# bdsaglam/torch-scae

Hardware: AMD Instinct MI355X
Metric: images/sec SCAE fwd+bwd, MNIST 40x40 bs=128, 1/2/4/8 MI355X (higher is better)
Workload: dtype f32

## Files before the change

include/scae_hip.h:

```cpp
#ifndef SCAE_HIP_H
#define SCAE_HIP_H

#include <stdint.h>

#ifdef __cplusplus
extern "C" {
#endif

#define SCAE_ABI_VERSION 3

#define SCAE_OK 0
#define SCAE_ERR_BAD_ARG (-1)
#define SCAE_ERR_UNSUPPORTED (-2)

#define SCAE_MAX_CHANNELS 4
#define SCAE_ATTN_MAX_SET 64
#define SCAE_RENDER_MAX_TEMPLATE_ELEMS 4096

int scae_abi_version(void);
const char *scae_error_string(int code);

void *scae_launch_list_begin(void *stream);
int scae_launch_list_end(void *list);
int scae_launch_list_size(const void *list);
// ... 30 lines not shown
                               float *gq, float *gk, float *gv,
                               float *gpresence, int HB, int N, int M, int dk,
                               int dv, float sqrt_dk, void *stream);

int scae_set_encoder_param_count(int D, int Din, int Dout, int L, int layer_norm);
int scae_set_encoder_grid(int B);
int scae_set_encoder_supported(int N, int D, int Din, int Dout, int L, int layer_norm);
int scae_set_encoder_fwd_f32(int nseg, const float *const *seg_ptr, const int *seg_width,
                             const int *seg_row_stride, const int64_t *seg_batch_stride,
                             const float *presence, const float *params, float *z,
                             float *hsave, int B, int N, int D, int Din, int Dout, int L,
                             int layer_norm, void *stream);
int scae_set_encoder_bwd_f32(int nseg, const float *const *seg_ptr, const int *seg_width,
                             const int *seg_row_stride, const int64_t *seg_batch_stride,
                             float *const *seg_grad, const float *presence,
                             const float *params, const float *hsave, const float *gz,
                             float *pg_partial, int B, int N, int D, int Din, int Dout,
                             int L, int layer_norm, void *stream);
int scae_set_encoder_bf16_supported(int N, int D, int Din, int Dout, int L, int layer_norm);
int scae_set_encoder_fwd_bf16(int nseg, const float *const *seg_ptr, const int *seg_width,
                              const int *seg_row_stride, const int64_t *seg_batch_stride,
                              const float *presence, const float *params, float *z,
                              float *hsave, int B, int N, int D, int Din, int Dout, int L,
                              int layer_norm, void *stream);
int scae_set_encoder_bwd_bf16(int nseg, const float *const *seg_ptr, const int *seg_width,
                              const int *seg_row_stride, const int64_t *seg_batch_stride,
                              float *const *seg_grad, const float *presence,
                              const float *params, const float *hsave, const float *gz,
                              float *pg_partial, int B, int N, int D, int Din, int Dout,
                              int L, int layer_norm, void *stream);

int scae_seed_attention_splits(int B, int O);
int scae_seed_attention_grid(int B, int O);
int scae_seed_attention_supported(int N, int O, int D, int C);
int scae_seed_attention_fwd_f32(const float *h, const float *q, const float *wk,
                                const float *bk, const float *wv, const float *bv,
                                const float *presence, float *out, float *probs, int B,
                                int N, int O, int D, int C, void *stream);
int scae_seed_attention_bwd_f32(const float *h, const float *q, const float *wk,
                                const float *bk, const float *wv, const float *bv,
                                const float *presence, const float *gout, float *gh,
                                float *partial, int B, int N, int O, int D, int C,
                                void *stream);

int scae_seed_attention_mfma_supported(int N, int O, int D, int C);
int scae_seed_attention_mfma_rows(int B);
int scae_seed_attention_mfma_fwd_f32(const float *h, const float *q, const float *wk,
                                     const float *wv, const float *bv, const float *presence,
                                     float *out, int B, int N, int O, int C, void *stream);
int scae_seed_attention_mfma_bwd_f32(const float *h, const float *q, const float *wk,
                                     const float *wv, const float *presence, const float *gout,
                                     float *gh, float *partial, int B, int N, int O, int C,
                                     void *stream);
int scae_seed_attention_mfma_fwd_bf16(const float *h, const float *q, const float *wk,
                                      const float *wv, const float *bv, const float *presence,
                                      float *out, int B, int N, int O, int C, void *stream);
int scae_seed_attention_mfma_bwd_bf16(const float *h, const float *q, const float *wk,
                                      const float *wv, const float *presence,
                                      const float *gout, float *gh, float *partial, int B,
                                      int N, int O, int C, void *stream);
int scae_seed_attention_mfma_reduce_f32(const float *partial, int rows, const float *q,
                                        const float *wk, float *gq, float *gwk, float *gbk,
                                        float *gwv, float *gbv, int O, int C, void *stream);

typedef struct scae_seed_fold_desc {
  const float *seeds;
  const float *wq, *bq, *wk, *bk, *wv, *bv, *wo, *bo;
  const float *w2, *b2;
  float *q, *wkf, *bkf, *wvf, *bvf;
  float *wv2e;
  float *wowv;
  int O, C, D;
} scae_seed_fold_desc;
typedef struct scae_seed_fold_grads {
  const float *g_q, *g_wkf, *g_bkf, *g_wvf, *g_bvf;
  float *d_seeds, *d_wq, *d_bq, *d_wk, *d_bk, *d_wv, *d_bv, *d_wo, *d_bo, *d_w2, *d_b2;
  float *gv2e, *t1;
} scae_seed_fold_grads;
int scae_seed_fold_supported(int O, int C, int D);
int scae_seed_fold_fwd_f32(const scae_seed_fold_desc *desc, void *stream);
int scae_seed_fold_bwd_f32(const scae_seed_fold_desc *desc, const scae_seed_fold_grads *grads,
                           void *stream);

int scae_layer_norm_rows(int64_t rows);
int scae_layer_norm_fwd_f32(const float *x, const float *weight, const float *bias, float *y,
                            float *mean, float *rstd, int64_t rows, int d, float eps,
                            void *stream);
int scae_layer_norm_bwd_f32(const float *x, const float *weight, const float *mean,
                            const float *rstd, const float *gy, float *gx, float *partial,
                            int64_t rows, int d, void *stream);

int scae_gemm_f32(const float *A, const float *B, float *C, const float *bias,
                  const float *mask, float *asum, int batch, int M, int N, int K,
                  int a_kcontig, int lda, int64_t a_batch, int b_kcontig, int ldb,
                  int64_t b_batch, int ldc, int64_t c_batch, int bias_ld, int64_t bias_batch,
                  int ldmask, int64_t mask_batch, int64_t asum_batch, int asum_ld, int relu,
                  void *stream);

typedef struct scae_gemm_desc {
  const float *A, *B;
  float *C;
  const float *bias, *mask;
  float *asum;
  int batch, M, N, K;
  int a_kcontig, lda;
  int64_t a_batch;
  int b_kcontig, ldb;
  int64_t b_batch;
  int ldc;
  int64_t c_batch;
  int bias_ld;
  int64_t bias_batch;
  int ldmask;
  int64_t mask_batch, asum_batch;
  int relu, asum_ld;
  float *c_nomask;
} scae_gemm_desc;
int scae_gemm_pair_f32(const scae_gemm_desc *first, const scae_gemm_desc *second, void *stream);
int scae_gemm_multi_f32(const scae_gemm_desc *descs, int n, void *stream);
int scae_seed_attention_mfma_bwd_gemm_f32(const float *h, const float *q, const float *wk,
                                          const float *wv, const float *presence,
                                          const float *gout, float *gh, float *partial, int B,
                                          int N, int O, int C, const scae_gemm_desc *descs,
                                          int n, void *stream);
int scae_seed_attention_mfma_bwd_gemm_bf16(const float *h, const float *q, const float *wk,
                                           const float *wv, const float *presence,
                                           const float *gout, float *gh, float *partial, int B,
                                           int N, int O, int C, const scae_gemm_desc *descs,
                                           int n, void *stream);


typedef struct scae_mlp_chain_layer {
  const float *w;
  int64_t w_gs;
  int ldw, K, N;
  const float *bias;
  int64_t bias_gs;
  int bias_ld;
  const float *gate;
  int64_t gate_gs, gate_bs;
  float *out;
  int64_t out_gs, out_bs;
  int relu;
} scae_mlp_chain_layer;
typedef struct scae_mlp_chain_desc {
  scae_mlp_chain_layer layer[4];
  int n_layers;
  const float *in;
  int64_t in_gs, in_bs;
  int in_dim, B, G;
  int row_tile;
  int bf16;
} scae_mlp_chain_desc;
int scae_mlp_chain_max_width(void);
int scae_mlp_chain_fwd_f32(const scae_mlp_chain_desc *desc, void *stream);
int scae_mlp_chain_bwd_f32(const scae_mlp_chain_desc *desc, void *stream);

typedef struct scae_votes_desc {
  const float *all_param;
  const float *cpr_static, *bias_cvr, *bias_caps, *bias_vote, *bias_scale;
  const float *noise_caps, *noise_vote;
  float noise_scale;
  int V, ld_param, similarity, learn_vote_scale, allow_deformations;
  float *vote, *scale, *vote_presence, *logit_caps, *logit_vote, *reg_partial;
  float *caps_presence;
  int *caps_arg;
  const float *gvote, *gscale, *gvote_presence, *glogit_caps, *glogit_vote, *greg;
  const float *gcaps_presence;
  float *gall_param, *gcpr_in, *gall_param_gated;
} scae_votes_desc;
int scae_mlp_chain_votes_fwd_f32(const scae_mlp_chain_desc *desc, const scae_votes_desc *votes,
                                 void *stream);
int scae_mlp_chain_votes_bwd_f32(const scae_mlp_chain_desc *desc, const scae_votes_desc *votes,
                                 void *stream);

int scae_gemm_bf16(const float *A, const float *B, float *C, const float *bias,
                   const float *mask, float *asum, int batch, int M, int N, int K,
                   int a_kcontig, int lda, int64_t a_batch, int b_kcontig, int ldb,
                   int64_t b_batch, int ldc, int64_t c_batch, int bias_ld, int64_t bias_batch,
                   int ldmask, int64_t mask_batch, int64_t asum_batch, int asum_ld, int relu,
                   void *stream);
int scae_gemm_pair_bf16(const scae_gemm_desc *first, const scae_gemm_desc *second, void *stream);
int scae_gemm_multi_bf16(const scae_gemm_desc *descs, int n, void *stream);
int scae_conv3x3_fwd_fold_f32(const float *in, const float *wf, const float *bias, float *out,
                              const float *post_bias, float *out_post, int B, int IH, int IW,
                              int Cin, int Cout, int stride, const scae_seed_fold_desc *fold,
                              void *stream);
int scae_conv3x3_fwd_res_supported(int B, int IH, int IW, int Cin, int Cout, int stride);
int scae_conv3x3_fwd_res_f32(const float *in, const float *wp, const float *bias, float *out,
                             const float *post_bias, float *out_post, int B, int IH, int IW,
                             int Cin, int Cout, int stride, int group, void *stream);
int scae_conv3x3_fwd_bf16(const float *in, const float *wf, const float *bias, float *out,
                          const float *post_bias, float *out_post, int B, int IH, int IW, int Cin,
                          int Cout, int stride, void *stream);
int scae_conv3x3_bwd_pair_bf16(const float *dpre, const float *wd, const float *in, float *din,
                               float *partial, int B, int IH, int IW, int Cin, int Cout,
                               int stride, void *stream);

int64_t scae_conv3x3_wf_floats(int Cout, int Cin);
int scae_conv3x3_relayout_f32(const float *w, float *wf, float *wd, int Cout, int Cin,
                              void *stream);

int scae_conv3x3_bf16r_supported(int B, int IH, int IW, int Cin, int Cout, int stride);
int scae_conv3x3_first_fwd_relayout_bf16(const float *img, const float *w, const float *bias,
                                         uint16_t *out_h, int B, int Cin, int IH, int IW,
                                         int Cout, int stride, int n_layers,
                                         const float *const *rw, float *const *rwf,
                                         float *const *rwd, uint16_t *const *rwfh,
                                         uint16_t *const *rwdh, const int *rCout,
                                         const int *rCin, void *stream);
int scae_cvt_bf16_batch(int n_arrays, const float *const *src, uint16_t *const *dst,
                        const int64_t *n, void *stream);
int scae_conv3x3_fwd_bf16r(const uint16_t *in, const uint16_t *wf, const float *bias,
                           uint16_t *out_h, float *out_f, const float *post_bias,
                           float *out_post, int B, int IH, int IW, int Cin, int Cout, int stride,
                           void *stream);
int scae_conv3x3_dgrad_bf16r(const uint16_t *dpre, const uint16_t *wd, const uint16_t *gate,
                             uint16_t *din_h, float *din_f, int B, int IH, int IW, int Cin,
                             int Cout, int stride, void *stream);
int scae_conv3x3_wgrad_bf16r_splits(int B, int OH, int OW, int Cin, int Cout);
int scae_conv3x3_wgrad_bf16r(const uint16_t *dpre, const uint16_t *x, float *partial, int B,
                             int IH, int IW, int Cin, int Cout, int stride, void *stream);
int scae_conv3x3_relayout_batch_f32(int n_layers, const float *const *w, float *const *wf,
                                    float *const *wd, const int *Cout, const int *Cin,
                                    void *stream);
int scae_conv3x3_first_fwd_f32(const float *img, const float *w, const float *bias,
                               float *out, int B, int Cin, int IH, int IW, int Cout,
                               int stride, void *stream);
int scae_conv3x3_first_wgrad_rows(int B, int Cout);
int scae_conv3x3_first_wgrad_f32(const float *dpre, const float *img, float *partial, int B,
                                 int Cin, int IH, int IW, int Cout, int stride, void *stream);
int scae_conv3x3_first_fwd_relayout_f32(const float *img, const float *w, const float *bias,
                                        float *out, int B, int Cin, int IH, int IW, int Cout,
                                        int stride, int n_layers, const float *const *rw,
                                        float *const *rwf, float *const *rwd, const int *rCout,
                                        const int *rCin, void *stream);
int scae_conv3x3_first_wgrad_reduce_f32(const float *dpre, const float *img, float *partial,
                                        int B, int Cin, int IH, int IW, int Cout, int stride,
                                        int n_layers, const float *const *rpartial,
                                        float *const *rdw, float *const *rdb, const int *rCout,
                                        const int *rCin, const int *rsplits, void *stream);
int scae_conv3x3_fwd_f32(const float *in, const float *wf, const float *bias, float *out,
                         const float *post_bias, float *out_post, int B, int IH, int IW,
                         int Cin, int Cout, int stride, void *stream);
int scae_conv3x3_dgrad_f32(const float *dpre, const float *wd, const float *gate, float *din,
                           int B, int IH, int IW, int Cin, int Cout, int stride, void *stream);
int scae_conv3x3_bwd_pair_f32(const float *dpre, const float *wd, const float *in, float *din,
                              float *partial, int B, int IH, int IW, int Cin, int Cout,
                              int stride, void *stream);
int scae_conv3x3_bwd_pair_reduce_f32(const float *dpre, const float *wd, const float *in,
                                     float *din, float *partial, int B, int IH, int IW, int Cin,
                                     int Cout, int stride, const float *rpartial, int rows,
                                     const float *q, const float *wk, float *gq, float *gwk,
                                     float *gbk, float *gwv, float *gbv, int O, int C,
                                     void *stream);
int scae_conv3x3_bwd_pair_fold_f32(const float *dpre, const float *wd, const float *in,
                                   float *din, float *partial, int B, int IH, int IW, int Cin,
                                   int Cout, int stride, const scae_seed_fold_desc *fold,
                                   const scae_seed_fold_grads *fold_grads, void *stream);
int scae_conv3x3_wgrad_splits(int B, int OH, int OW, int Cin, int Cout);
int scae_conv3x3_wgrad_f32(const float *dpre, const float *in, float *partial, float *dw,
                           float *db, int B, int IH, int IW, int Cin, int Cout, int stride,
                           void *stream);
int scae_conv3x3_wgrad_reduce_batch_f32(int n_layers, const float *const *partial,
                                        float *const *dw, float *const *db, const int *Cout,
                                        const int *Cin, const int *splits, void *stream);

int scae_attention_pool_supported(int HW, int A, int P);
int scae_attention_pool_fwd_f32(const float *y, float *out, int B, int HW, int A, int P,
                                void *stream);
int scae_attention_pool_bwd_f32(const float *y, const float *g, float *dy, int B, int HW,
                                int A, int P, void *stream);
int scae_capsule_head_fwd_f32(const float *y, const float *noise_u, float noise_scale,
                              int similarity, float *pooled, float *pose, float *presence,
                              float *feature, float *absence, int B, int HW, int A, int P,
                              void *stream);
int scae_capsule_head_conv_supported(int HW, int A, int P, int C);
int scae_capsule_head_conv_preferred(int B, int HW, int A, int P, int C);
int scae_capsule_head_conv_fwd_f32(const float *x, const float *w, const float *bias, int C,
                                   float *y, const float *noise_u, float noise_scale,
                                   int similarity, float *pooled, float *pose, float *presence,
                                   float *feature, float *absence, int B, int HW, int A, int P,
                                   void *stream);
int scae_capsule_head_conv_fwd_tc_f32(
    const float *x, const float *w, const float *bias, int C, float *y, const float *noise_u,
    float noise_scale, int similarity, float *pooled, float *pose, float *presence,
    float *feature, float *absence, int B, int HW, int A, int P, const float *logits,
    const float *w1, const float *b1, const float *w2, const float *b2, float *raw,
    float *templates, float *color, int Ct, int hw, int F, int H1, int template_nonlin,
    int color_nonlin, void *stream);
int scae_capsule_head_bwd_f32(const float *y, const float *pooled, const float *noise_u,
                              float noise_scale, int similarity, const float *g_pose,
                              const float *g_presence, const float *g_feature,
                              const float *g_feature2, float *dy, int B, int HW, int A, int P,
                              void *stream);
int scae_capsule_head_bwd_tc_f32(
    const float *y, const float *pooled, const float *noise_u, float noise_scale, int similarity,
    const float *g_pose, const float *g_presence, const float *g_feature, float *dy, int B,
    int HW, int A, int P, const float *logits, const float *feature, const float *w1,
    const float *b1, const float *w2, const float *b2, const float *color,
    const float *g_templates, const float *g_raw, float *g_logits, float *tc_g_feature,
    float *partial, int C, int hw, int F, int H1, int template_nonlin, int color_nonlin,
    void *stream);

int scae_rmsprop_step_f32(float *param, const float *grad, float *square_avg, float *buf,
                          int64_t n, float lr, const float *lr_dev, float alpha, float eps,
                          float momentum, float weight_decay, float grad_scale, void *stream);

struct scae_sum_job;
int scae_rmsprop_sums_step_f32(float *param, float *grad, float *square_avg, float *buf,
                               int64_t n, float lr, const float *lr_dev, float alpha, float eps,
                               float momentum, float grad_scale, const struct scae_sum_job *jobs,
                               int n_jobs, void *stream);

#define SCAE_FLAT_OPT_STATE_INTS 2112
int scae_flat_opt_step_f32(float *param, const float *grad, float *exp_avg, float *exp_avg_sq,
                           float *slow, int64_t n, const float *lr_dev, int32_t *step_state,
                           int kind, double beta1, double beta2, float eps, float weight_decay,
                           float grad_scale, int look_ahead_k, float look_ahead_alpha,
                           int advance, void *stream);

int scae_flat_opt_sums_step_f32(float *param, float *grad, float *exp_avg, float *exp_avg_sq,
                                float *slow, int64_t n, const float *lr_dev,
                                int32_t *step_state, int kind, double beta1, double beta2,
                                float eps, float grad_scale, int look_ahead_k,
                                float look_ahead_alpha, const struct scae_sum_job *jobs,
                                int n_jobs, void *stream);

#define SCAE_GRAD_SQ_MAX_PARTIALS 4096
int scae_grad_sq_partials_f32(const float *grad, int64_t n, double *partials, int max_partials,
                              int *n_partials, void *stream);

int scae_grad_sq_partials_sums_f32(float *grad, int64_t n, double *partials, int max_partials,
                                   int *n_partials, const struct scae_sum_job *jobs, int n_jobs,
                                   void *stream);

int scae_rmsprop_clip_step_f32(float *param, const float *grad, float *square_avg, float *buf,
                               int64_t n, float lr, const float *lr_dev, float alpha, float eps,
                               float momentum, float weight_decay, float grad_scale,
                               const double *partials, int n_partials, float max_norm,
                               float *norm_out, void *stream);
int scae_flat_opt_clip_step_f32(float *param, const float *grad, float *exp_avg,
                                float *exp_avg_sq, float *slow, int64_t n, const float *lr_dev,
                                int32_t *step_state, int kind, double beta1, double beta2,
                                float eps, float weight_decay, float grad_scale,
                                int look_ahead_k, float look_ahead_alpha, int advance,
                                const double *partials, int n_partials, float max_norm,
                                float *norm_out, void *stream);

int scae_grad_accumulate_f32(float *acc, const float *grad, int64_t n, void *stream);
int scae_grad_accumulate_sums_f32(float *acc, float *grad, int64_t n,
                                  const struct scae_sum_job *jobs, int n_jobs, void *stream);
int scae_grad_sq_acc_partials_f32(const float *grad, const float *acc, int64_t n,
                                  double *partials, int max_partials, int *n_partials,
                                  void *stream);
int scae_grad_sq_acc_partials_sums_f32(float *grad, const float *acc, int64_t n,
                                       double *partials, int max_partials, int *n_partials,
                                       const struct scae_sum_job *jobs, int n_jobs,
                                       void *stream);
int scae_rmsprop_acc_step_f32(float *param, const float *grad, float *acc, float *square_avg,
                              float *buf, int64_t n, float lr, const float *lr_dev, float alpha,
                              float eps, float momentum, float weight_decay, float grad_scale,
                              void *stream);
int scae_rmsprop_acc_sums_step_f32(float *param, float *grad, float *acc, float *square_avg,
                                   float *buf, int64_t n, float lr, const float *lr_dev,
                                   float alpha, float eps, float momentum, float grad_scale,
                                   const struct scae_sum_job *jobs, int n_jobs, void *stream);
int scae_rmsprop_acc_clip_step_f32(float *param, const float *grad, float *acc,
                                   float *square_avg, float *buf, int64_t n, float lr,
                                   const float *lr_dev, float alpha, float eps, float momentum,
                                   float weight_decay, float grad_scale, const double *partials,
                                   int n_partials, float max_norm, float *norm_out,
                                   void *stream);
int scae_flat_opt_acc_step_f32(float *param, const float *grad, float *acc, float *exp_avg,
                               float *exp_avg_sq, float *slow, int64_t n, const float *lr_dev,
                               int32_t *step_state, int kind, double beta1, double beta2,
                               float eps, float weight_decay, float grad_scale,
                               int look_ahead_k, float look_ahead_alpha, int advance,
                               void *stream);
int scae_flat_opt_acc_sums_step_f32(float *param, float *grad, float *acc, float *exp_avg,
                                    float *exp_avg_sq, float *slow, int64_t n,
                                    const float *lr_dev, int32_t *step_state, int kind,
                                    double beta1, double beta2, float eps, float grad_scale,
                                    int look_ahead_k, float look_ahead_alpha,
                                    const struct scae_sum_job *jobs, int n_jobs, void *stream);
int scae_flat_opt_acc_clip_step_f32(float *param, const float *grad, float *acc,
                                    float *exp_avg, float *exp_avg_sq, float *slow, int64_t n,
                                    const float *lr_dev, int32_t *step_state, int kind,
                                    double beta1, double beta2, float eps, float weight_decay,
                                    float grad_scale, int look_ahead_k, float look_ahead_alpha,
                                    int advance, const double *partials, int n_partials,
                                    float max_norm, float *norm_out, void *stream);

#define SCAE_NORM_CHUNK 2048
#define SCAE_NORM_GROUP_CHUNKS 16
#define SCAE_NORM_INF 0
int scae_segment_norms_chunk(void);
int scae_segment_norms_f32(const float *src, const float *acc, int64_t n, const int32_t *chunks,
                           int n_chunks, const int32_t *group_first, int n_groups,
                           const int32_t *seg_first, int n_segs, int norm_kind, float scale,
                           double *partials, float *ring, int64_t *cursor, int capacity,
                           void *stream);

int scae_stage_batch(float *dst_image, const float *src_image, int64_t n_image,
                     int64_t *dst_label, const int64_t *src_label, int64_t n_label,
                     void *stream);

int scae_step_prologue_f32(float *dst_image, const float *src_image, int64_t n_image,
                           int64_t *dst_label, const int64_t *src_label, int64_t n_label,
                           float *noise, int64_t n_noise, uint64_t *noise_state,
                           const scae_seed_fold_desc *fold, void *stream);

typedef struct scae_first_layer_desc {
  const float *img;
  const float *w;
  const float *bias;
  float *out;
  int B, Cin, IH, IW, Cout, stride;
  int n_layers;
  const float *rw[8];
  float *rwf[8];
  float *rwd[8];
  int rCout[8], rCin[8];
  uint16_t *out_h;
  uint16_t *rwfh[8];
  uint16_t *rwdh[8];
} scae_first_layer_desc;
int scae_step_prologue_first_f32(float *dst_image, const float *src_image, int64_t n_image,
                                 int64_t *dst_label, const int64_t *src_label,
                                 int64_t n_label, float *noise, int64_t n_noise,
                                 uint64_t *noise_state, const scae_seed_fold_desc *fold,
                                 const scae_first_layer_desc *first, void *stream);

typedef struct scae_batch_source_desc {
  const void *images;
  const void *labels;
  const int32_t *index;
  int64_t rows;
  int64_t n;
  int image_u8, label_u8;
  int C, h, w, H, W;
  int shuffle, translate;
  uint64_t seed;
  int64_t epoch, position;
  int rank, world;
  int wrap;
  const int32_t *affine;
  int64_t affine_rows;
} scae_batch_source_desc;
int scae_gather_batch_f32(float *dst_image, int64_t *dst_label, int B,
                          const scae_batch_source_desc *src, void *stream);
int scae_step_prologue_source_f32(float *dst_image, int64_t *dst_label, int B,
                                  const scae_batch_source_desc *src, float *noise,
                                  int64_t n_noise, uint64_t *noise_state,
                                  const scae_seed_fold_desc *fold,
                                  const scae_first_layer_desc *first, void *stream);

int scae_template_color_supported(int M, int C, int F, int H1);
int scae_template_color_partial_rows(int B, int M);
int scae_template_color_fwd_f32(const float *logits, const float *feature, const float *w1,
                                const float *b1, const float *w2, const float *b2, float *raw,
                                float *templates, float *color, int B, int M, int C, int hw,
                                int F, int H1, int template_nonlin, int color_nonlin,
                                void *stream);
int scae_template_color_bwd_f32(const float *logits, const float *feature, const float *w1,
                                const float *b1, const float *w2, const float *b2,
                                const float *color, const float *g_templates,
                                const float *g_raw, float *g_logits, float *g_feature,
                                float *partial, int B, int M, int C, int hw, int F, int H1,
                                int template_nonlin, int color_nonlin, void *stream);

typedef struct scae_sum_segment {
  float *dst;
  int64_t begin, end, period;
} scae_sum_segment;
int scae_sum_rows_f32(const float *src, int64_t rows, int64_t cols,
                      const scae_sum_segment *segments, int n_segments, void *stream);
typedef struct scae_sum_job {
  const float *src;
  int64_t rows, cols;
  const scae_sum_segment *segments;
  int n_segments;
} scae_sum_job;
int scae_sum_rows_multi_f32(const scae_sum_job *jobs, int n_jobs, void *stream);

typedef struct scae_scaled_sum {
  const float *src;
  int64_t n;
  float scale;
  float *dst;
} scae_scaled_sum;
int scae_scaled_sums_f32(const scae_scaled_sum *jobs, int n_jobs, void *stream);

int scae_capsule_votes_fwd_f32(const float *all_param, const float *cpr_static,
                               const float *bias_cvr, const float *bias_caps,
                               const float *bias_vote, const float *bias_scale,
                               const float *noise_caps, const float *noise_vote,
                               float noise_scale, float *vote, float *scale,
                               float *vote_presence, float *logit_caps,
                               float *logit_vote, float *reg_partial,
                               float *caps_presence, int *caps_arg, int B, int O, int V,
                               int ld_param, int similarity, int learn_vote_scale,
                               int allow_deformations, void *stream);
int scae_capsule_votes_bwd_f32(const float *all_param, const float *cpr_static,
                               const float *bias_cvr, const float *bias_caps,
                               const float *bias_vote, const float *bias_scale,
                               const float *noise_caps, const float *noise_vote,
                               float noise_scale, const float *gvote,
                               const float *gscale, const float *gvote_presence,
                               const float *glogit_caps, const float *glogit_vote,
                               const float *greg, const float *gcaps_presence,
                               const int *caps_arg, float *gall_param, float *gcpr_in,
                               float *gall_param_gated, int B, int O, int V, int ld_param,
                               int similarity, int learn_vote_scale,
                               int allow_deformations, void *stream);

int scae_capsule_likelihood_fwd_f32(
    const float *vote, const float *scale, const float *vote_presence,
    const float *dummy_vote, const float *x, const float *presence,
    float *log_prob_per_point, float *vote_presence_binary, float *winner,
    float *winner_presence, int64_t *winner_idx, int64_t *is_from_capsule,
    float *soft_winner, float *soft_winner_presence, float *posterior,
    float *mixing_log_prob, float *mixing_logit, int B, int O, int M,
    void *stream);
int scae_capsule_likelihood_bwd_f32(
    const float *vote, const float *scale, const float *vote_presence,
    const float *dummy_vote, const float *x, const float *presence,
    const float *posterior, const int64_t *winner_idx, const float *g_lpp,
    const float *g_winner, const float *g_winner_presence,
    const float *g_soft_winner, const float *g_soft_winner_presence,
    const float *g_posterior, const float *g_mixing_log_prob,
    const float *g_mixing_logit, float *gvote, float *gscale,
    float *gvote_presence, float *gx, float *gpresence, float *gdummy_partial,
    int B, int O, int M, void *stream);

int scae_class_probs_supported(int O, int ncls);
int scae_class_probs_f32(const float *caps_presence, const float *posterior, const float *w,
                         const float *bias, float *prior_prob, float *post_prob, int B, int O,
                         int M, int ncls, const scae_scaled_sum *extra_sums, int n_extra,
                         void *stream);

typedef struct scae_eval_sink {
  float *rows;
  int64_t capacity;
  int64_t cursor;
  int64_t overflow;
} scae_eval_sink;
#define SCAE_EVAL_RECORD_FLOATS 9
#define SCAE_EVAL_RECORDS_MAX_CLASSES 64
typedef struct scae_eval_records {
  float *rows;
  int64_t capacity;
  int64_t cursor;
  int64_t overflow;
  int64_t *confusion;
  int64_t ncls;
  int64_t labelled;
} scae_eval_records;
#define SCAE_TRAIN_LOG_ROW 19
typedef struct scae_train_log_desc {
  float *rows;
  int64_t *step;
  int capacity;
  double *acc;
  const float *prior_prob, *post_prob;
  const int64_t *label;
  int ncls;
  const float *lr;
} scae_train_log_desc;
typedef struct scae_loss_extras {
  const float *rec_sums;
  int n_rec;
  const float *reg;
  float w_reg;
  float *g_rec_sums, *g_reg;
  float *loss;
  const float *g_loss;
  int defer_combine;
  float *out12;
  const scae_train_log_desc *train_log;
} scae_loss_extras;
int scae_loss_tail_supported(int B, int O, int ncls);
int64_t scae_loss_tail_workspace_floats(int B, int O, int ncls);
int scae_loss_tail_fwd_f32(const float *lpp, const float *posterior,
                           const float *caps_presence, const float *cls_w,
                           const float *cls_b, const int64_t *label,
                           const scae_loss_extras *extras, float *out12, float *workspace,
                           int B, int O, int M, int ncls, int n_classes_cfg, int prior_type,
                           int post_type, int sparsity_on, const float *weights5,
                           float within_const, void *stream);
int scae_loss_tail_defer_preferred(int B, int O);
int scae_loss_tail_combine_f32(const float *lpp, const float *posterior,
                               const float *caps_presence, const float *cls_w,
                               const float *cls_b, const int64_t *label,
                               const scae_loss_extras *extras, float *out12, float *workspace,
                               int B, int O, int M, int ncls, int n_classes_cfg, int prior_type,
                               int post_type, int sparsity_on, const float *weights5,
                               float within_const, void *stream);
int scae_loss_tail_fwd_class_probs_f32(
    const float *lpp, const float *posterior, const float *caps_presence, const float *cls_w,
    const float *cls_b, const int64_t *label, const scae_loss_extras *extras, float *out12,
    float *workspace, int B, int O, int M, int ncls, int n_classes_cfg, int prior_type,
    int post_type, int sparsity_on, const float *weights5, float within_const,
    const float *cp_caps_presence, const float *cp_posterior, const float *cp_w,
    const float *cp_bias, float *prior_prob, float *post_prob, int cp_B, int cp_O, int cp_M,
    int cp_ncls, const scae_scaled_sum *extra_sums, int n_extra, void *stream);
// ... 313 lines not shown
```

torch_scae_amd/_lib.py:

```python
import ctypes
import os
from ctypes import (POINTER, Structure, c_char_p, c_double, c_float, c_int,
                    c_int64, c_uint32, c_uint64, c_void_p)

_HERE = os.path.dirname(os.path.abspath(__file__))
LIB_PATH = os.environ.get("SCAE_HIP_LIB") or os.path.join(_HERE, "lib",
                                                        "libscae_hip.so")

P = c_void_p


class DecoderDesc(Structure):
    _fields_ = [("templates", P), ("templates_alpha", P), ("pose", P),
                ("presence", P), ("bg_image", P), ("bg_value", P),
                ("bg_mixing_logit", P), ("temperature_logit", P),
                ("out_scale", P),
                ("B", c_int), ("M", c_int), ("C", c_int), ("th", c_int),
                ("tw", c_int), ("H", c_int), ("W", c_int),
                ("template_repeat", c_int)]


class LikelihoodBwdDesc(Structure):
    _fields_ = [(n, P) for n in (
        "vote", "scale", "vote_presence", "dummy_vote", "x", "presence",
        "posterior", "winner_idx", "g_lpp", "g_winner", "g_winner_presence",
        "g_soft_winner", "g_soft_winner_presence", "g_posterior",
        "g_mixing_log_prob", "g_mixing_logit", "gvote", "gscale",
        "gvote_presence", "gx", "gpresence", "gdummy_partial")] + [
        ("B", c_int), ("O", c_int), ("M", c_int)]


class GemmDesc(Structure):
    _fields_ = [("A", P), ("B", P), ("C", P), ("bias", P), ("mask", P),
                ("asum", P), ("batch", c_int), ("M", c_int), ("N", c_int),
                ("K", c_int), ("a_kcontig", c_int), ("lda", c_int),
                ("a_batch", c_int64), ("b_kcontig", c_int), ("ldb", c_int),
                ("b_batch", c_int64), ("ldc", c_int), ("c_batch", c_int64),
                ("bias_ld", c_int), ("bias_batch", c_int64), ("ldmask", c_int),
                ("mask_batch", c_int64), ("asum_batch", c_int64),
                ("relu", c_int), ("asum_ld", c_int), ("c_nomask", P)]


class MlpChainLayer(Structure):
    _fields_ = [("w", P), ("w_gs", c_int64), ("ldw", c_int), ("K", c_int),
                ("N", c_int), ("bias", P), ("bias_gs", c_int64),
                ("bias_ld", c_int), ("gate", P), ("gate_gs", c_int64),
                ("gate_bs", c_int64), ("out", P), ("out_gs", c_int64),
                ("out_bs", c_int64), ("relu", c_int)]


class MlpChainDesc(Structure):
    _fields_ = [("layer", MlpChainLayer * 4), ("n_layers", c_int), ("in_", P),
                ("in_gs", c_int64), ("in_bs", c_int64), ("in_dim", c_int),
                ("B", c_int), ("G", c_int), ("row_tile", c_int),
                ("bf16", c_int)]


class VotesDesc(Structure):
    _fields_ = [(n, P) for n in ("all_param", "cpr_static", "bias_cvr",
                                 "bias_caps", "bias_vote", "bias_scale",
                                 "noise_caps", "noise_vote")] + \
        [("noise_scale", c_float), ("V", c_int), ("ld_param", c_int),
         ("similarity", c_int), ("learn_vote_scale", c_int),
         ("allow_deformations", c_int)] + \
        [(n, P) for n in ("vote", "scale", "vote_presence", "logit_caps",
                          "logit_vote", "reg_partial", "caps_presence",
                          "caps_arg", "gvote", "gscale", "gvote_presence",
                          "glogit_caps", "glogit_vote", "greg", "gcaps_presence",
                          "gall_param", "gcpr_in", "gall_param_gated")]


class SumSegment(Structure):
    _fields_ = [("dst", P), ("begin", c_int64), ("end", c_int64),
                ("period", c_int64)]


class SumJob(Structure):
    _fields_ = [("src", P), ("rows", c_int64), ("cols", c_int64),
                ("segments", POINTER(SumSegment)), ("n_segments", c_int)]


class ScaledSum(Structure):
    _fields_ = [("src", P), ("n", c_int64), ("scale", c_float), ("dst", P)]


class TrainLogDesc(Structure):
    _fields_ = [("rows", P), ("step", P), ("capacity", c_int), ("acc", P),
                ("prior_prob", P), ("post_prob", P), ("label", P), ("ncls", c_int),
                ("lr", P)]


class LossExtras(Structure):
    _fields_ = [("rec_sums", P), ("n_rec", c_int), ("reg", P),
                ("w_reg", c_float), ("g_rec_sums", P), ("g_reg", P),
                ("loss", P), ("g_loss", P), ("defer_combine", c_int),
                ("out12", P), ("train_log", POINTER(TrainLogDesc))]


class KMeansDesc(Structure):
    _fields_ = [("x", P), ("N", c_int64), ("F", c_int), ("k", c_int), ("R", c_int),
                ("G", c_int), ("max_iter", c_int), ("centroids", P), ("labels", P),
                ("part_sum", P), ("part_count", P), ("part_changed", P),
                ("part_inertia", P), ("state", P), ("inertia", P)]


class ProbeDesc(Structure):
    _fields_ = [("x", P), ("y", P), ("N", c_int64), ("F", c_int), ("C", c_int), ("R", c_int),
                ("G", c_int), ("max_iter", c_int), ("mean", P), ("scale", P), ("l2", P),
                ("step", P), ("tol", P), ("W", P), ("V", P), ("grad", P), ("t", P),
                ("part_grad", P), ("part_loss", P), ("history", P), ("state", P)]


class TsneDesc(Structure):
    _fields_ = [("N", c_int), ("G", c_int), ("n_iter", c_int), ("exaggeration_iter", c_int),
                ("check_every", c_int), ("early_exaggeration", c_float),
                ("learning_rate", c_float), ("P", P), ("Y", P), ("velocity", P), ("gains", P),
                ("part", P), ("rows", P), ("block", P), ("plogp", P), ("history", P)]


class TsneSparseDesc(Structure):
    _fields_ = [("N", c_int), ("G", c_int), ("n_iter", c_int), ("exaggeration_iter", c_int),
                ("check_every", c_int), ("early_exaggeration", c_float),
                ("learning_rate", c_float), ("indptr", P), ("cols", P), ("vals", P),
                ("nnz", c_int64), ("Y", P), ("velocity", P), ("gains", P), ("part", P),
                ("rows", P), ("block", P), ("plogp", P), ("history", P)]


class SeedFoldDesc(Structure):
    _fields_ = [(n, P) for n in (
        "seeds", "wq", "bq", "wk", "bk", "wv", "bv", "wo", "bo", "w2", "b2",
        "q", "wkf", "bkf", "wvf", "bvf", "wv2e", "wowv")] + \
        [("O", c_int), ("C", c_int), ("D", c_int)]


class FirstLayerDesc(Structure):
    _fields_ = [("img", P), ("w", P), ("bias", P), ("out", P)] + \
        [(n, c_int) for n in ("B", "Cin", "IH", "IW", "Cout", "stride",
                              "n_layers")] + \
        [("rw", P * 8), ("rwf", P * 8), ("rwd", P * 8),
         ("rCout", c_int * 8), ("rCin", c_int * 8),
         ("out_h", P), ("rwfh", P * 8), ("rwdh", P * 8)]


class BatchSourceDesc(Structure):
    _fields_ = [("images", P), ("labels", P), ("index", P), ("rows", c_int64),
                ("n", c_int64)] + \
        [(n, c_int) for n in ("image_u8", "label_u8", "C", "h", "w", "H", "W",
                              "shuffle", "translate")] + \
        [("seed", c_uint64), ("epoch", c_int64), ("position", c_int64),
         ("rank", c_int), ("world", c_int), ("wrap", c_int),
         ("affine", P), ("affine_rows", c_int64)]


class SeedFoldGrads(Structure):
    _fields_ = [(n, P) for n in (
        "g_q", "g_wkf", "g_bkf", "g_wvf", "g_bvf", "d_seeds", "d_wq", "d_bq",
        "d_wk", "d_bk", "d_wv", "d_bv", "d_wo", "d_bo", "d_w2", "d_b2",
        "gv2e", "t1")]


SIGNATURES = {
    "scae_abi_version": [],
    "scae_error_string": [c_int],
    "scae_uniform_f32": [P, c_int64, P, P],
    "scae_geometric_transform_fwd_f32": [P, P, c_int64, c_int, c_int, c_int, P],
    "scae_geometric_transform_bwd_f32": [P, P, P, c_int64, c_int, c_int, c_int,
                                         P],
    "scae_mat3_mul_fwd_f32": [P, P, P, c_int64, c_int, P],
    "scae_mat3_mul_bwd_f32": [P, P, P, P, P, c_int64, c_int, P],
    "scae_qkv_attention_fwd_f32": [P, P, P, P, P, P, c_int, c_int, c_int,
                                   c_int, c_int, c_float, P],
    "scae_qkv_attention_fwd_bf16": [P, P, P, P, P, P, c_int, c_int, c_int,
                                    c_int, c_int, c_float, P],
    "scae_qkv_attention_bwd_f32": [P, P, P, P, P, P, P, P, P, c_int, c_int,
                                   c_int, c_int, c_int, c_float, P],
    "scae_set_encoder_param_count": [c_int] * 5,
    "scae_set_encoder_grid": [c_int],
    "scae_set_encoder_supported": [c_int] * 6,
    "scae_set_encoder_fwd_f32": [c_int, P, P, P, P, P, P, P, P] + [c_int] * 7 + [P],
    "scae_set_encoder_bwd_f32": [c_int, P, P, P, P, P, P, P, P, P, P]
                                + [c_int] * 7 + [P],
    "scae_render_gmm_sums_bwd_likelihood_f32": [P] * 13,
    "scae_set_encoder_fwd_logprob_f32": [c_int, P, P, P, P, P, P, P, P] + [c_int] * 7
                                        + [P] * 6,
    "scae_set_encoder_fwd_logprob_bf16": [c_int, P, P, P, P, P, P, P, P] + [c_int] * 7
                                         + [P] * 6,
    "scae_set_encoder_bf16_supported": [c_int] * 6,
    "scae_set_encoder_fwd_bf16": [c_int, P, P, P, P, P, P, P, P] + [c_int] * 7 + [P],
    "scae_set_encoder_bwd_bf16": [c_int, P, P, P, P, P, P, P, P, P, P]
                                 + [c_int] * 7 + [P],
    "scae_seed_attention_splits": [c_int] * 2,
    "scae_seed_attention_grid": [c_int] * 2,
    "scae_seed_attention_supported": [c_int] * 4,
    "scae_seed_attention_fwd_f32": [P] * 9 + [c_int] * 5 + [P],
    "scae_seed_attention_bwd_f32": [P] * 10 + [c_int] * 5 + [P],
    "scae_seed_attention_mfma_supported": [c_int] * 4,
    "scae_seed_attention_mfma_rows": [c_int],
    "scae_seed_attention_mfma_fwd_f32": [P] * 7 + [c_int] * 4 + [P],
    "scae_seed_attention_mfma_bwd_f32": [P] * 8 + [c_int] * 4 + [P],
    "scae_seed_attention_mfma_fwd_bf16": [P] * 7 + [c_int] * 4 + [P],
    "scae_seed_attention_mfma_bwd_bf16": [P] * 8 + [c_int] * 4 + [P],
    "scae_seed_attention_mfma_bwd_gemm_f32": [P] * 8 + [c_int] * 4
    + [POINTER(GemmDesc), c_int, P],
    "scae_seed_attention_mfma_bwd_gemm_bf16": [P] * 8 + [c_int] * 4
    + [POINTER(GemmDesc), c_int, P],
    "scae_seed_attention_mfma_reduce_f32": [P, c_int] + [P] * 7 + [c_int] * 2 + [P],
    "scae_seed_fold_supported": [c_int] * 3,
    "scae_seed_fold_fwd_f32": [POINTER(SeedFoldDesc), P],
    "scae_seed_fold_bwd_f32": [POINTER(SeedFoldDesc), POINTER(SeedFoldGrads), P],
    "scae_layer_norm_rows": [c_int64],
    "scae_layer_norm_fwd_f32": [P] * 6 + [c_int64, c_int, c_float, P],
    "scae_layer_norm_bwd_f32": [P] * 7 + [c_int64, c_int, P],
    "scae_gemm_f32": [P] * 6 + [c_int] * 6 + [c_int64, c_int, c_int, c_int64,
                                              c_int, c_int64, c_int, c_int64,
                                              c_int, c_int64, c_int64, c_int, c_int,
                                              P],
    "scae_gemm_bf16": [P] * 6 + [c_int] * 6 + [c_int64, c_int, c_int, c_int64,
                                              c_int, c_int64, c_int, c_int64,
                                              c_int, c_int64, c_int64, c_int, c_int,
                                              P],
    "scae_gemm_pair_f32": [POINTER(GemmDesc), POINTER(GemmDesc), P],
    "scae_launch_list_begin": [P],
    "scae_launch_list_end": [P],
    "scae_launch_list_size": [P],
    "scae_launch_list_run": [P, P],
    "scae_launch_list_lane": [P, c_int],
    "scae_launch_list_timeline": [P, P, P, POINTER(c_float), c_int],
    "scae_launch_list_free": [P],
    "scae_gemm_multi_f32": [POINTER(GemmDesc), c_int, P],
    "scae_gemm_multi_bf16": [POINTER(GemmDesc), c_int, P],
    "scae_mlp_chain_max_width": [],
    "scae_mlp_chain_fwd_f32": [POINTER(MlpChainDesc), P],
    "scae_mlp_chain_bwd_f32": [POINTER(MlpChainDesc), P],
    "scae_mlp_chain_votes_fwd_f32": [POINTER(MlpChainDesc), POINTER(VotesDesc), P],
    "scae_mlp_chain_votes_bwd_f32": [POINTER(MlpChainDesc), POINTER(VotesDesc), P],
    "scae_gemm_pair_bf16": [POINTER(GemmDesc), POINTER(GemmDesc), P],
    "scae_conv3x3_wf_floats": [c_int, c_int],
    "scae_conv3x3_relayout_f32": [P, P, P, c_int, c_int, P],
    "scae_conv3x3_bf16r_supported": [c_int] * 6,
    "scae_conv3x3_first_fwd_relayout_bf16": [P] * 4 + [c_int] * 7 + [P] * 8,
    "scae_cvt_bf16_batch": [c_int, P, P, P, P],
    "scae_conv3x3_fwd_bf16r": [P] * 7 + [c_int] * 6 + [P],
    "scae_conv3x3_dgrad_bf16r": [P] * 5 + [c_int] * 6 + [P],
    "scae_conv3x3_wgrad_bf16r_splits": [c_int] * 5,
    "scae_conv3x3_wgrad_bf16r": [P] * 3 + [c_int] * 6 + [P],
    "scae_conv3x3_relayout_batch_f32": [c_int, P, P, P, P, P, P],
    "scae_conv3x3_first_fwd_f32": [P] * 4 + [c_int] * 6 + [P],
    "scae_conv3x3_first_fwd_relayout_f32": [P] * 4 + [c_int] * 7 + [P] * 6,
    "scae_conv3x3_first_wgrad_reduce_f32": [P] * 3 + [c_int] * 7 + [P] * 7,
    "scae_conv3x3_first_wgrad_rows": [c_int] * 2,
    "scae_conv3x3_first_wgrad_f32": [P] * 3 + [c_int] * 6 + [P],
    "scae_conv3x3_fwd_f32": [P] * 6 + [c_int] * 6 + [P],
    "scae_conv3x3_fwd_fold_f32": [P] * 6 + [c_int] * 6 + [POINTER(SeedFoldDesc), P],
    "scae_conv3x3_fwd_res_supported": [c_int] * 6,
    "scae_conv3x3_fwd_res_f32": [P] * 6 + [c_int] * 7 + [P],
    "scae_conv3x3_fwd_bf16": [P] * 6 + [c_int] * 6 + [P],
    "scae_conv3x3_dgrad_f32": [P] * 4 + [c_int] * 6 + [P],
    "scae_conv3x3_bwd_pair_f32": [P] * 5 + [c_int] * 6 + [P],
    "scae_conv3x3_bwd_pair_reduce_f32": [P] * 5 + [c_int] * 6 + [P, c_int] + [P] * 7
    + [c_int] * 2 + [P],
    "scae_conv3x3_bwd_pair_fold_f32": [P] * 5 + [c_int] * 6
    + [POINTER(SeedFoldDesc), POINTER(SeedFoldGrads), P],
    "scae_conv3x3_bwd_pair_bf16": [P] * 5 + [c_int] * 6 + [P],
    "scae_conv3x3_wgrad_reduce_batch_f32": [c_int] + [P] * 7,
    "scae_conv3x3_wgrad_splits": [c_int] * 5,
    "scae_conv3x3_wgrad_f32": [P] * 5 + [c_int] * 6 + [P],
    "scae_attention_pool_supported": [c_int] * 3,
    "scae_attention_pool_fwd_f32": [P, P] + [c_int] * 4 + [P],
    "scae_attention_pool_bwd_f32": [P, P, P] + [c_int] * 4 + [P],
    "scae_stage_batch": [P, P, c_int64, P, P, c_int64, P],
    "scae_step_prologue_f32": [P, P, c_int64, P, P, c_int64, P, c_int64, P,
                               POINTER(SeedFoldDesc), P],
    "scae_step_prologue_first_f32": [P, P, c_int64, P, P, c_int64, P, c_int64,
                                     P, POINTER(SeedFoldDesc),
                                     POINTER(FirstLayerDesc), P],
    "scae_gather_batch_f32": [P, P, c_int, POINTER(BatchSourceDesc), P],
    "scae_step_prologue_source_f32": [P, P, c_int, POINTER(BatchSourceDesc), P, c_int64, P,
                                      POINTER(SeedFoldDesc), POINTER(FirstLayerDesc), P],
    "scae_rmsprop_step_f32": [P, P, P, P, c_int64, c_float, P, c_float, c_float,
                              c_float, c_float, c_float, P],
    "scae_rmsprop_sums_step_f32": [P, P, P, P, c_int64, c_float, P, c_float, c_float,
                                   c_float, c_float, POINTER(SumJob), c_int, P],
    "scae_flat_opt_step_f32": [P, P, P, P, P, c_int64, P, P, c_int, c_double, c_double, c_float,
                               c_float, c_float, c_int, c_float, c_int, P],
    "scae_flat_opt_sums_step_f32": [P, P, P, P, P, c_int64, P, P, c_int, c_double, c_double,
                                    c_float, c_float, c_int, c_float, POINTER(SumJob), c_int, P],
    "scae_grad_sq_partials_f32": [P, c_int64, P, c_int, POINTER(c_int), P],
    "scae_grad_sq_partials_sums_f32": [P, c_int64, P, c_int, POINTER(c_int), POINTER(SumJob),
                                       c_int, P],
    "scae_rmsprop_clip_step_f32": [P, P, P, P, c_int64, c_float, P, c_float, c_float, c_float,
                                   c_float, c_float, P, c_int, c_float, P, P],
    "scae_flat_opt_clip_step_f32": [P, P, P, P, P, c_int64, P, P, c_int, c_double, c_double,
                                    c_float, c_float, c_float, c_int, c_float, c_int, P, c_int,
                                    c_float, P, P],
    "scae_grad_accumulate_f32": [P, P, c_int64, P],
    "scae_grad_accumulate_sums_f32": [P, P, c_int64, POINTER(SumJob), c_int, P],
    "scae_grad_sq_acc_partials_f32": [P, P, c_int64, P, c_int, POINTER(c_int), P],
    "scae_grad_sq_acc_partials_sums_f32": [P, P, c_int64, P, c_int, POINTER(c_int),
                                           POINTER(SumJob), c_int, P],
    "scae_rmsprop_acc_step_f32": [P, P, P, P, P, c_int64, c_float, P, c_float, c_float,
                                  c_float, c_float, c_float, P],
    "scae_rmsprop_acc_sums_step_f32": [P, P, P, P, P, c_int64, c_float, P, c_float, c_float,
                                       c_float, c_float, POINTER(SumJob), c_int, P],
    "scae_rmsprop_acc_clip_step_f32": [P, P, P, P, P, c_int64, c_float, P, c_float, c_float,
                                       c_float, c_float, c_float, P, c_int, c_float, P, P],
    "scae_flat_opt_acc_step_f32": [P, P, P, P, P, P, c_int64, P, P, c_int, c_double, c_double,
                                   c_float, c_float, c_float, c_int, c_float, c_int, P],
    "scae_flat_opt_acc_sums_step_f32": [P, P, P, P, P, P, c_int64, P, P, c_int, c_double,
                                        c_double, c_float, c_float, c_int, c_float,
                                        POINTER(SumJob), c_int, P],
    "scae_flat_opt_acc_clip_step_f32": [P, P, P, P, P, P, c_int64, P, P, c_int, c_double,
                                        c_double, c_float, c_float, c_float, c_int, c_float,
                                        c_int, P, c_int, c_float, P, P],
    "scae_segment_norms_chunk": [],
    "scae_segment_norms_f32": [P, P, c_int64, P, c_int, P, c_int, P, c_int, c_int, c_float,
                               P, P, P, c_int, P],
    "scae_capsule_head_fwd_f32": [P, P, c_float, c_int, P, P, P, P, P] + [c_int] * 4 + [P],
    "scae_capsule_head_conv_supported": [c_int] * 4,
    "scae_capsule_head_conv_preferred": [c_int] * 5,
    "scae_capsule_head_conv_fwd_f32": [P, P, P, c_int, P, P, c_float, c_int, P, P, P, P, P]
    + [c_int] * 4 + [P],
    "scae_capsule_head_conv_fwd_tc_f32": [P, P, P, c_int, P, P, c_float, c_int, P, P, P, P, P]
    + [c_int] * 4 + [P] * 8 + [c_int] * 6 + [P],
    "scae_capsule_head_bwd_f32": [P, P, P, c_float, c_int, P, P, P, P, P] + [c_int] * 4 + [P],
    "scae_capsule_head_bwd_tc_f32": [P, P, P, c_float, c_int, P, P, P, P] + [c_int] * 4
    + [P] * 12 + [c_int] * 6 + [P],
    "scae_template_color_supported": [c_int] * 4,
    "scae_template_color_partial_rows": [c_int] * 2,
    "scae_template_color_fwd_f32": [P] * 9 + [c_int] * 8 + [P],
    "scae_template_color_bwd_f32": [P] * 12 + [c_int] * 8 + [P],
    "scae_sum_rows_f32": [P, c_int64, c_int64, POINTER(SumSegment), c_int, P],
    "scae_sum_rows_multi_f32": [POINTER(SumJob), c_int, P],
    "scae_scaled_sums_f32": [POINTER(ScaledSum), c_int, P],
    "scae_class_probs_supported": [c_int] * 2,
    "scae_class_probs_f32": [P] * 6 + [c_int] * 4 + [POINTER(ScaledSum), c_int, P],
    "scae_capsule_votes_fwd_f32": [P] * 8 + [c_float] + [P] * 8
                                  + [c_int] * 7 + [P],
    "scae_capsule_votes_bwd_f32": [P] * 8 + [c_float] + [P] * 11
                                  + [c_int] * 7 + [P],
    "scae_capsule_likelihood_fwd_f32": [P] * 17 + [c_int] * 3 + [P],
    "scae_capsule_likelihood_bwd_f32": [P] * 22 + [c_int] * 3 + [P],
    "scae_loss_tail_supported": [c_int] * 3,
    "scae_loss_tail_workspace_floats": [c_int] * 3,
    "scae_loss_tail_fwd_f32": [P] * 6 + [POINTER(LossExtras), P, P] + [c_int] * 8
    + [POINTER(c_float), c_float, P],
    "scae_loss_tail_defer_preferred": [c_int] * 2,
    "scae_loss_tail_combine_f32": [P] * 6 + [POINTER(LossExtras), P, P] + [c_int] * 8
    + [POINTER(c_float), c_float, P],
    "scae_loss_tail_fwd_class_probs_f32": [P] * 6 + [POINTER(LossExtras), P, P]
    + [c_int] * 8 + [POINTER(c_float), c_float] + [P] * 6 + [c_int] * 4
    + [POINTER(ScaledSum), c_int, P],
    "scae_loss_tail_bwd_f32": [P] * 6 + [POINTER(LossExtras)] + [P] * 7
    + [c_int] * 8 + [POINTER(c_float), c_float, P],
    "scae_eval_tail_f32": [P] * 6 + [POINTER(LossExtras), P, P] + [c_int] * 8
    + [POINTER(c_float), c_float] + [P] * 5,
    "scae_loss_tail_fwd_class_probs_sink_f32": [P] * 6 + [POINTER(LossExtras), P, P]
    + [c_int] * 8 + [POINTER(c_float), c_float] + [P] * 6 + [c_int] * 4
    + [POINTER(ScaledSum), c_int, P, P],
    "scae_eval_tail_sink_f32": [P] * 6 + [POINTER(LossExtras), P, P] + [c_int] * 8
    + [POINTER(c_float), c_float] + [P] * 6,
    "scae_eval_tail_records_f32": [P] * 6 + [POINTER(LossExtras), P, P] + [c_int] * 8
    + [POINTER(c_float), c_float] + [P] * 7,
    "scae_eval_records_f32": [P] * 6 + [c_int] * 4 + [P, P],
    "scae_eval_accumulate_f32": [P] * 5 + [c_int] * 2 + [P] * 3,
    "scae_train_log_f32": [P] * 3 + [POINTER(TrainLogDesc), c_int, P],
    "scae_eval_features_f32": [P, P, c_int, c_int, c_int, P, P],
    "scae_kmeans_supported": [c_int] * 2,
    "scae_kmeans_groups": [c_int64, c_int],
    "scae_kmeans_lloyd_f32": [POINTER(KMeansDesc), c_int, P],
    "scae_kmeans_pp_f32": [P, c_int64, c_int, c_int, c_int, c_uint32, P, P, P, P],
    "scae_kmeans_assign_f32": [P, c_int64, c_int, c_int, P, P, P],
    "scae_kmeans_contingency": [P, P, c_int64, c_int, c_int, P, P, P],
    "scae_probe_supported": [c_int] * 3,
    "scae_probe_groups": [c_int64, c_int],
    "scae_probe_predict_blocks": [c_int64],
    "scae_probe_moments_f64": [P, P, c_int64, c_int, c_int, P, P, P, P],
    "scae_probe_fit_f32": [POINTER(ProbeDesc), c_int, P],
    "scae_probe_predict_f32": [P, c_int64, c_int, c_int] + [P] * 8,
    "scae_tsne_supported": [c_int] * 2,
    "scae_tsne_groups": [c_int],
    "scae_tsne_affinities_f32": [P, c_int, c_int, c_float, P, P, P, P, P],
    "scae_tsne_run_f32": [POINTER(TsneDesc), c_int, c_int, P],
    "scae_tsne_sparse_supported": [c_int] * 3,
    "scae_tsne_sparse_groups": [c_int],
    "scae_tsne_knn_bandwidths_f32": [P, c_int, c_int, c_float, P, P, P],
    "scae_tsne_sparse_run_f32": [POINTER(TsneSparseDesc), c_int, c_int, P],
    "scae_knn_wide_f32": [P, c_int64, c_int, c_int, P, P, P, P],
    "scae_knn_supported": [c_int64, c_int64, c_int, c_int],
    "scae_knn_groups": [c_int64, c_int64],
    "scae_knn_f32": [P, c_int64, P, c_int64, c_int, c_int, c_int, P, P, P, P],
    "scae_knn_vote_f32": [P, P, c_int64, c_int, P, c_int64, POINTER(c_int), c_int, c_int, P, P],
    "scae_knn_ranks_f32": [P, c_int64, c_int, P, c_int, P, P, P, P, P],
    "scae_cluster_quality_supported": [c_int64, c_int, c_int64],
    "scae_cluster_quality_labels": [P, c_int64, c_int64, P, P, P],
    "scae_cluster_quality_silhouette_f32": [P, P, P, P, c_int64, c_int, c_int64] + [P] * 7,
    "scae_cluster_quality_dispersion_f32": [P, P, c_int64, c_int, c_int64, P, P],
    "scae_template_render_fwd_f32": [POINTER(DecoderDesc), P, P, P],
    "scae_render_gmm_logprob_fwd_f32": [POINTER(DecoderDesc), P, P, P, P, P],
    "scae_render_gmm_bwd_f32": [POINTER(DecoderDesc)] + [P] * 12 + [P],
    "scae_render_gmm_logprob_tiles": [POINTER(DecoderDesc)],
    "scae_render_gmm_forms": [POINTER(DecoderDesc), c_int, P, P, POINTER(c_int)],
    "scae_render_gmm_logprob_sums_fwd_f32": [POINTER(DecoderDesc)] + [P] * 4 + [P],
    "scae_render_gmm_sums_bwd_f32": [POINTER(DecoderDesc)] + [P] * 10 + [P],
    "scae_gmm_log_prob_fwd_f32": [P] * 5 + [c_int] * 4 + [c_int64, P],
    "scae_gmm_log_prob_bwd_f32": [P] * 9 + [c_int] * 4 + [c_int64, P],
    "scae_gmm_mean_f32": [P] * 3 + [c_int] * 4 + [c_int64, P],
    "scae_gmm_mode_f32": [P] * 4 + [c_int] * 5 + [c_int64, P],
    "scae_render_gmm_mode_f32": [POINTER(DecoderDesc), P, c_int, c_int, c_int, P],
    "scae_render_gmm_parts_f32": [POINTER(DecoderDesc), P, P, P, c_int] + [P] * 7 + [c_int, c_int, P],
    "scae_render_gmm_parts_geometry": [POINTER(DecoderDesc), c_int, POINTER(c_int)],
    "scae_image_sheet_f32": [c_int, POINTER(P), POINTER(c_int)] + [c_int] * 5 + [c_float, P, P],
}

_RESTYPES = {"scae_error_string": c_char_p,
             "scae_loss_tail_workspace_floats": c_int64,
             "scae_conv3x3_wf_floats": c_int64,
             "scae_launch_list_begin": P,
             "scae_launch_list_free": None}
EVAL_ACC_DOUBLES = 17
TRAIN_LOG_ROW = 19
KMEANS_STATE_INTS = 4
PROBE_STATE_INTS = 4
TSNE_MAX_N = 32768
TSNE_MAX_F = 256
TSNE_HISTORY_COLS = 3
TSNE_BLOCK_DOUBLES = 640
TSNE_MAX_NEIGHBORS = 128
TSNE_SPARSE_MAX_N = 262144
TSNE_SPARSE_BLOCK_DOUBLES = 5120
KNN_MAX_K = 64
KNN_MAX_F = 256
KNN_MAX_KS = 8
CLUSTER_QUALITY_MAX_F = 256
EVAL_SINK_INT64S = 4
EVAL_RECORDS_INT64S = 7
EVAL_RECORD_FLOATS = 9
EVAL_RECORDS_MAX_CLASSES = 64
FLAT_OPT_STATE_INTS = 2112
GRAD_SQ_MAX_PARTIALS = 4096
NORM_CHUNK = 2048
NORM_GROUP_CHUNKS = 16
NORM_INF = 0
ABI_VERSION = 3

_lib = None


class ScaeHipError(RuntimeError):
    pass


def load():
    global _lib
    if _lib is not None:
        return _lib
    if not os.path.exists(LIB_PATH):
        raise ScaeHipError(
            f"{LIB_PATH} is missing: build it with `python -c 'import "
            f"__graft_entry__ as g; g.build()'` or `make -C torch_scae_amd/csrc`."
            " torch_scae_amd has no CPU / eager fallback.")
    lib = ctypes.CDLL(LIB_PATH)
    for name, argtypes in SIGNATURES.items():
        fn = getattr(lib, name)
        fn.argtypes = argtypes
        fn.restype = _RESTYPES.get(name, c_int)
        if argtypes and argtypes[-1] is P and not name.startswith("scae_launch_list"):
            setattr(lib, name, _recording(fn))
    if lib.scae_abi_version() != ABI_VERSION:
        raise ScaeHipError(
            f"{LIB_PATH} has ABI version {lib.scae_abi_version()}, this package "
            f"binds version {ABI_VERSION}: rebuild it (make -C torch_scae_amd/csrc)")
    _lib = lib
    return lib


_RECORDER = None


def _recording(fn):
    def launcher(*args):
        rc = fn(*args)
        if _RECORDER is not None and rc == 0:
            conv = []
            for t, a in zip(fn.argtypes, args):
                if a is None or isinstance(a, (int, float)):
                    a = t(a) if a is not None else t()
                conv.append(a)
            _RECORDER.append((fn, tuple(conv[:-1]), args))
        return rc
    launcher.__name__ = getattr(fn, "__name__", "launcher")
    return launcher


class recorder:

    def __enter__(self):
        global _RECORDER
        self.prev, self.launches = _RECORDER, []
        _RECORDER = self.launches
        return self.launches

    def __exit__(self, *exc):
        global _RECORDER
        _RECORDER = self.prev
        return False


def replay(launches, stream):
    for fn, cargs, _keep in launches:
        rc = fn(*cargs, stream)
        if rc != 0:
            check(rc, getattr(fn, "__name__", "launch"))


ERR_UNSUPPORTED = -2


def check(rc, what):
    if rc != 0:
        msg = load().scae_error_string(rc)
        raise ScaeHipError(f"{what} failed with code {rc}: "
                           f"{msg.decode() if msg else '?'}")


def call(name, *args):
    check(getattr(load(), name)(*args), name)


def try_call(name, *args):
    rc = getattr(load(), name)(*args)
    if rc == ERR_UNSUPPORTED:
        return False
    check(rc, name)
    return True
```

torch_scae_amd/csrc/attention_pool.hip:

```cpp
#include "geometric_transform.h"
#include "wave_mfma.h"

#define SCAE_DEVICE_ONLY
namespace scae_tc {
#include "template_color.hip"
}
#undef SCAE_DEVICE_ONLY

namespace {
constexpr int NT = 512;

struct PoolArgs {
  const float *y, *g;
  float *out, *dy;
  int B, HW, A, P;
  int splits;
  const float *noise_u;
  float noise_scale;
  int similarity;
  float *pose, *presence, *feature;
  float *absence;
  const float *pooled, *g_pose, *g_presence, *g_feature, *g_feature2;
  const float *cx, *cw, *cb;
  float *cy;
  int C;
};

__host__ __device__ inline int padded(int AP) { return AP | 1; }
inline int pool_splits(int B, int A) {
  int s = 1;
  for (int d = 1; d <= A && d <= 8; ++d)
    if (A % d == 0) {
      s = d;
      if ((long)B * d >= 512) break;
    }
  return s;
}
inline size_t lds_floats(int HW, int A, int P, bool bwd) {
  size_t n = (size_t)HW * padded(A * P) + (size_t)A * HW;
  n += bwd ? (size_t)A * HW + (size_t)A * (P - 1) + A
           : (size_t)A * (P - 1);
  return n;
}

__device__ __forceinline__ void stage_y(float *ys, const float *y, int HW, int AP, int APp,
                                        int ldy) {
  if ((AP & 3) == 0 && (ldy & 3) == 0 && ((size_t)y & 15) == 0) {
    const int q = AP / 4;
    for (int e = threadIdx.x; e < HW * q; e += NT) {
      const int pix = e / q, ch = 4 * (e - pix * q);
      const float4 v = *reinterpret_cast<const float4 *>(y + (size_t)pix * ldy + ch);
      float *d = ys + pix * APp + ch;
      d[0] = v.x, d[1] = v.y, d[2] = v.z, d[3] = v.w;
    }
  } else {
    for (int e = threadIdx.x; e < HW * AP; e += NT) {
      const int pix = e / AP, ch = e - pix * AP;
      ys[pix * APp + ch] = y[(size_t)pix * ldy + ch];
    }
  }
}

template <int NB>
__device__ __forceinline__ void conv_y(float *ys, float *xs, const PoolArgs &k, int b, int a0,
                                       int AP, int APp, int ldy) {
  using namespace scae_wave;
  constexpr int C = 64 * NB, XS = C + 4, q4 = C / 4;
  const int HW = k.HW;
  const int lane = threadIdx.x & 63, wave = threadIdx.x >> 6, r = lane & 15, q = lane >> 4;
  const int ncol = (AP + 15) / 16, nrow = (HW + 15) / 16;
  float4 wf[4 * NB];
  auto load_w = [&](int col) {
    const int ch = col * 16 + r;
    const float *wr = k.cw + (size_t)(a0 * k.P + (ch < AP ? ch : AP - 1)) * C + 4 * q;
#pragma unroll
    for (int t = 0; t < 4 * NB; ++t) wf[t] = ld4(wr + 16 * t);
  };
  if (wave < ncol) load_w(wave);
  const float *x = k.cx + (size_t)b * HW * C;
  for (int e = threadIdx.x; e < HW * q4; e += NT) {
    const int pix = e / q4, c = 4 * (e - pix * q4);
    *reinterpret_cast<float4 *>(xs + pix * XS + c) = ld4(x + (size_t)pix * C + c);
  }
  __syncthreads();
  float *y = k.cy + (size_t)b * HW * ldy + a0 * k.P;
  for (int col = wave; col < ncol; col += NT / 64) {
    if (col != wave) load_w(col);
    const int ch = col * 16 + r;
    const float bias = (k.cb && ch < AP) ? k.cb[a0 * k.P + ch] : 0.f;
    for (int rt = 0; rt < nrow; ++rt) {
      const int pix = rt * 16 + r;
      const float *xr = xs + (pix < HW ? pix : HW - 1) * XS + 4 * q;
      f32x4 acc = splat(0.f);
#pragma unroll
      for (int t = 0; t < 4 * NB; ++t) acc = mma16(acc, ld4(xr + 16 * t), wf[t]);
      if (ch < AP) {
#pragma unroll
        for (int j = 0; j < 4; ++j) {
          const int p = rt * 16 + 4 * q + j;
          if (p < HW) {
            const float v = acc[j] + bias;
            ys[p * APp + ch] = v;
            y[(size_t)p * ldy + ch] = v;
          }
        }
      }
    }
  }
}
inline bool conv_y_supported(int HW, int C) { return HW <= 32 && C >= 64 && C % 64 == 0 && C <= 256; }
__host__ __device__ inline int conv_x_offset(int HW, int A, int P) {
  return (HW * padded(A * P) + A * HW + A * (P - 1) + 3) & ~3;
}

__device__ __forceinline__ void softmax_masks(float *mask, const float *ys, int HW, int A, int P,
                                              int APp) {
  for (int t = threadIdx.x; t < ((A * 32 + NT - 1) / NT) * NT; t += NT) {
    const int a = t >> 5, l = t & 31;
    const bool ok = a < A;
    const float *col = ys + (ok ? a : 0) * P + P - 1;
    float mx = -INFINITY;
    if (ok)
      for (int pix = l; pix < HW; pix += 32) mx = fmaxf(mx, col[pix * APp]);
    mx = scae::row_max16(mx);
    mx = fmaxf(mx, __shfl_xor(mx, 16, 64));
    float s = 0.f;
    if (ok)
      for (int pix = l; pix < HW; pix += 32) {
        const float e = expf(col[pix * APp] - mx);
        mask[a * HW + pix] = e;
        s += e;
      }
    s = scae::row_sum16(s);
    s += __shfl_xor(s, 16, 64);
    const float inv = 1.f / s;
    if (ok)
      for (int pix = l; pix < HW; pix += 32) mask[a * HW + pix] *= inv;
  }
}

__device__ __forceinline__ void pool_fwd_body(const PoolArgs &k, float *lds, int blk) {
  const int Af = k.A, A = Af / k.splits, b = blk / k.splits, a0 = (blk % k.splits) * A;
  const int HW = k.HW, P = k.P, AP = A * P, APp = padded(AP), ldy = Af * P;
  const size_t cap0 = (size_t)b * Af + a0;
  float *ys = lds, *mask = ys + HW * APp;
  float *pooled = mask + A * HW;
  if (k.cx) {
    float *xs = lds + conv_x_offset(HW, A, P);
    switch (k.C / 64) {
      case 1: conv_y<1>(ys, xs, k, b, a0, AP, APp, ldy); break;
      case 2: conv_y<2>(ys, xs, k, b, a0, AP, APp, ldy); break;
      case 3: conv_y<3>(ys, xs, k, b, a0, AP, APp, ldy); break;
      default: conv_y<4>(ys, xs, k, b, a0, AP, APp, ldy); break;
    }
  } else
    stage_y(ys, k.y + (size_t)b * HW * ldy + a0 * P, HW, AP, APp, ldy);
  __syncthreads();
  softmax_masks(mask, ys, HW, A, P, APp);
  __syncthreads();
  for (int e = threadIdx.x; e < A * (P - 1); e += NT) {
    const int a = e / (P - 1), p = e - a * (P - 1);
    float s = 0.f;
    for (int pix = 0; pix < HW; ++pix) s = fmaf(ys[pix * APp + a * P + p], mask[a * HW + pix], s);
    k.out[cap0 * (P - 1) + e] = s;
    if (k.pose) pooled[e] = s;
  }
  if (!k.pose) return;
  __syncthreads();
  const int F = P - 8;
  for (int a = threadIdx.x; a < A; a += NT) {
    const float *row = pooled + a * (P - 1);
    scae_gt::GtState st;
    scae_gt::gt_eval(row, 1, st);
    float o[6];
    scae_gt::gt_rows(st, k.similarity, o);
#pragma unroll
    for (int j = 0; j < 6; ++j) k.pose[(cap0 + a) * 6 + j] = o[j];
    float logit = row[6];
    if (k.noise_u) logit += (k.noise_u[cap0 + a] - .5f) * k.noise_scale;
    const float pr = scae::sigmoidf_(logit);
    k.presence[cap0 + a] = pr;
    if (k.absence) k.absence[cap0 + a] = 1.f - pr;
  }
  if (k.feature)
    for (int e = threadIdx.x; e < A * F; e += NT) {
      const int a = e / F, f = e - a * F;
      k.feature[cap0 * F + e] = pooled[a * (P - 1) + 7 + f];
    }
}
__global__ __launch_bounds__(NT) void pool_fwd_kernel(PoolArgs k) {
  extern __shared__ __align__(16) float lds[];
  pool_fwd_body(k, lds, blockIdx.x);
}

__global__ __launch_bounds__(NT) void pool_tc_fwd_kernel(PoolArgs k, scae_tc::TcArgs tk) {
  extern __shared__ __align__(16) float lds[];
  pool_fwd_body(k, lds, blockIdx.x);
  __threadfence_block();
  __syncthreads();
  scae_tc::tc_fwd_body<NT>(tk, lds, blockIdx.x);
}

__device__ __forceinline__ void pool_bwd_body(const PoolArgs &k, float *lds, int blk) {
  const int Af = k.A, A = Af / k.splits, b = blk / k.splits, a0 = (blk % k.splits) * A;
  const int HW = k.HW, P = k.P, AP = A * P, APp = padded(AP), ldy = Af * P;
  const size_t cap0 = (size_t)b * Af + a0;
  float *ys = lds, *mask = ys + HW * APp, *t = mask + A * HW, *gs = t + A * HW,
        *sa = gs + A * (P - 1);
  stage_y(ys, k.y + (size_t)b * HW * ldy + a0 * P, HW, AP, APp, ldy);
  if (k.pooled) {
    const int F = P - 8;
    for (int a = threadIdx.x; a < A; a += NT) {
      const float *row = k.pooled + (cap0 + a) * (P - 1);
      float raw[6], go[6], gp[6];
#pragma unroll
      for (int j = 0; j < 6; ++j) {
        raw[j] = row[j];
        go[j] = k.g_pose ? k.g_pose[(cap0 + a) * 6 + j] : 0.f;
      }
      scae_gt::GtState st;
      scae_gt::gt_eval(raw, 1, st);
      scae_gt::gt_backward(st, k.similarity, go, gp);
#pragma unroll
      for (int j = 0; j < 6; ++j) gs[a * (P - 1) + j] = gp[j];
      float logit = row[6];
      if (k.noise_u) logit += (k.noise_u[cap0 + a] - .5f) * k.noise_scale;
      const float sg = scae::sigmoidf_(logit);
      gs[a * (P - 1) + 6] = k.g_presence ? k.g_presence[cap0 + a] * sg * (1.f - sg) : 0.f;
    }
    for (int e = threadIdx.x; e < A * F; e += NT) {
      const int a = e / F, f = e - a * F;
      gs[a * (P - 1) + 7 + f] = (k.g_feature ? k.g_feature[cap0 * F + e] : 0.f) +
                                (k.g_feature2 ? k.g_feature2[cap0 * F + e] : 0.f);
    }
  } else {
    for (int e = threadIdx.x; e < A * (P - 1); e += NT) gs[e] = k.g[cap0 * (P - 1) + e];
  }
  __syncthreads();
  softmax_masks(mask, ys, HW, A, P, APp);
  for (int e = threadIdx.x; e < A * HW; e += NT) {
    const int a = e / HW, pix = e - a * HW;
    float s = 0.f;
    for (int p = 0; p < P - 1; ++p) s = fmaf(gs[a * (P - 1) + p], ys[pix * APp + a * P + p], s);
    t[e] = s;
  }
  __syncthreads();
  for (int u = threadIdx.x; u < ((A * 32 + NT - 1) / NT) * NT; u += NT) {
    const int a = u >> 5, l = u & 31;
    float s = 0.f;
    if (a < A)
      for (int pix = l; pix < HW; pix += 32) s = fmaf(mask[a * HW + pix], t[a * HW + pix], s);
    s = scae::row_sum16(s);
    s += __shfl_xor(s, 16, 64);
    if (a < A && l == 0) sa[a] = s;
  }
  __syncthreads();
  float *dy = k.dy + (size_t)b * HW * ldy + a0 * P;
  for (int e = threadIdx.x; e < HW * AP; e += NT) {
    const int pix = e / AP, ch = e - pix * AP, a = ch / P, p = ch - a * P;
    const float m = mask[a * HW + pix];
    dy[(size_t)pix * ldy + ch] =
        p < P - 1 ? gs[a * (P - 1) + p] * m : m * (t[a * HW + pix] - sa[a]);
  }
}
__global__ __launch_bounds__(NT) void pool_bwd_kernel(PoolArgs k) {
  extern __shared__ float lds[];
  pool_bwd_body(k, lds, blockIdx.x);
}

__global__ __launch_bounds__(NT) void pool_tc_bwd_kernel(PoolArgs k, scae_tc::TcArgs tk, int nA) {
  extern __shared__ __attribute__((aligned(16))) float lds[];
  if ((int)blockIdx.x >= nA) {
    scae_tc::tc_bwdB_body<NT>(tk, (int)blockIdx.x - nA);
    return;
  }
  scae_tc::tc_bwdA_body<NT>(tk, lds, blockIdx.x);
  __syncthreads();
  pool_bwd_body(k, lds, blockIdx.x);
}

int check(const PoolArgs &k) {
  if (k.B <= 0 || k.HW <= 0 || k.A <= 0 || k.P < 2) return SCAE_ERR_BAD_ARG;
  if (!scae_attention_pool_supported(k.HW, k.A, k.P)) return SCAE_ERR_UNSUPPORTED;
  return SCAE_OK;
}
}

extern "C" int scae_capsule_head_bwd_tc_f32(
    const float *y, const float *pooled, const float *noise_u, float noise_scale, int similarity,
    const float *g_pose, const float *g_presence, const float *g_feature, float *dy, int B,
    int HW, int A, int P, const float *logits, const float *feature, const float *w1,
    const float *b1, const float *w2, const float *b2, const float *color,
    const float *g_templates, const float *g_raw, float *g_logits, float *tc_g_feature,
    float *partial, int C, int hw, int F, int H1, int template_nonlin, int color_nonlin,
    void *stream) {
  PoolArgs k{};
  k.y = y, k.dy = dy, k.B = B, k.HW = HW, k.A = A, k.P = P;
  k.splits = pool_splits(B, A);
  k.noise_u = noise_u, k.noise_scale = noise_scale, k.similarity = similarity;
  k.pooled = pooled, k.g_pose = g_pose, k.g_presence = g_presence, k.g_feature = g_feature;
  k.g_feature2 = tc_g_feature;
  int rc = check(k);
  if (rc) return rc;
  if (P < 8) return SCAE_ERR_UNSUPPORTED;
  SCAE_REQUIRE(y && pooled && dy);
  scae_tc::TcArgs tk;
  rc = scae_tc::bwd_args(tk, logits, feature, w1, b1, w2, b2, color, g_templates, g_raw, g_logits,
                         tc_g_feature, partial, B, A, C, hw, F, H1, template_nonlin,
                         color_nonlin);
  if (rc) return rc;
  if (tk.splits != k.splits || F != P - 8) return SCAE_ERR_UNSUPPORTED;
  if (k.splits == 1) return SCAE_ERR_UNSUPPORTED;
  const size_t lp = lds_floats(HW, A / k.splits, P, true),
               lt = scae_tc::lds_floats(A / k.splits, C, F, H1, true);
  const int nA = B * k.splits;
  scae::launch(pool_tc_bwd_kernel, dim3(nA + scae_tc::bwd_elementwise_blocks(tk)), dim3(NT),
                     (lp > lt ? lp : lt) * sizeof(float), (hipStream_t)stream, k, tk, nA);
  return scae_launch_status();
}

extern "C" int scae_attention_pool_supported(int HW, int A, int P) {
  if (HW <= 0 || A <= 0 || P < 2) return 0;
  return lds_floats(HW, A, P, true) * sizeof(float) <= 128 * 1024;
}

extern "C" int scae_attention_pool_fwd_f32(const float *y, float *out, int B, int HW, int A,
                                           int P, void *stream) {
  PoolArgs k{};
  k.y = y, k.out = out, k.B = B, k.HW = HW, k.A = A, k.P = P;
  k.splits = pool_splits(B, A);
  int rc = check(k);
  if (rc) return rc;
  SCAE_REQUIRE(y && out);
  scae::launch(pool_fwd_kernel, dim3(B * k.splits), dim3(NT),
                     lds_floats(HW, A / k.splits, P, false) * sizeof(float),
                     (hipStream_t)stream, k);
  return scae_launch_status();
}

extern "C" int scae_attention_pool_bwd_f32(const float *y, const float *g, float *dy, int B,
                                           int HW, int A, int P, void *stream) {
  PoolArgs k{};
  k.y = y, k.g = g, k.dy = dy, k.B = B, k.HW = HW, k.A = A, k.P = P;
  k.splits = pool_splits(B, A);
  int rc = check(k);
  if (rc) return rc;
  SCAE_REQUIRE(y && g && dy);
  scae::launch(pool_bwd_kernel, dim3(B * k.splits), dim3(NT),
                     lds_floats(HW, A / k.splits, P, true) * sizeof(float),
                     (hipStream_t)stream, k);
  return scae_launch_status();
}

extern "C" int scae_capsule_head_fwd_f32(const float *y, const float *noise_u, float noise_scale,
                                         int similarity, float *pooled, float *pose,
                                         float *presence, float *feature, float *absence, int B,
                                         int HW, int A, int P, void *stream) {
  PoolArgs k{};
  k.y = y, k.out = pooled, k.B = B, k.HW = HW, k.A = A, k.P = P;
  k.splits = pool_splits(B, A);
  k.noise_u = noise_u, k.noise_scale = noise_scale, k.similarity = similarity;
  k.pose = pose, k.presence = presence, k.feature = feature, k.absence = absence;
  int rc = check(k);
  if (rc) return rc;
  if (P < 8) return SCAE_ERR_UNSUPPORTED;
  SCAE_REQUIRE(y && pooled && pose && presence && (feature || P == 8));
  scae::launch(pool_fwd_kernel, dim3(B * k.splits), dim3(NT),
                     lds_floats(HW, A / k.splits, P, false) * sizeof(float),
                     (hipStream_t)stream, k);
  return scae_launch_status();
}

extern "C" int scae_capsule_head_conv_supported(int HW, int A, int P, int C) {
  return scae_attention_pool_supported(HW, A, P) && P >= 8 && conv_y_supported(HW, C);
}

extern "C" int scae_capsule_head_conv_preferred(int B, int HW, int A, int P, int C) {
  if (B <= 0 || !scae_capsule_head_conv_supported(HW, A, P, C)) return 0;
  const int group = A / pool_splits(B, A);
  return (size_t)B * A * P * C * sizeof(float) <= ((size_t)48 << 20) &&
         (group * P + 15) / 16 <= 2 * (NT / 64);
}

extern "C" int scae_capsule_head_conv_fwd_f32(const float *x, const float *w, const float *bias,
                                              int C, float *y, const float *noise_u,
                                              float noise_scale, int similarity, float *pooled,
                                              float *pose, float *presence, float *feature,
                                              float *absence, int B, int HW, int A, int P,
                                              void *stream) {
  PoolArgs k{};
  k.cx = x, k.cw = w, k.cb = bias, k.cy = y, k.C = C;
  k.out = pooled, k.B = B, k.HW = HW, k.A = A, k.P = P;
  k.splits = pool_splits(B, A);
  k.noise_u = noise_u, k.noise_scale = noise_scale, k.similarity = similarity;
  k.pose = pose, k.presence = presence, k.feature = feature, k.absence = absence;
  int rc = check(k);
  if (rc) return rc;
  if (!scae_capsule_head_conv_supported(HW, A, P, C)) return SCAE_ERR_UNSUPPORTED;
  SCAE_REQUIRE(x && w && y && pooled && pose && presence && (feature || P == 8));
  SCAE_REQUIRE((((size_t)x | (size_t)w) & 15) == 0);
  const int Ag = A / k.splits;
  scae::launch(pool_fwd_kernel, dim3(B * k.splits), dim3(NT),
                     (conv_x_offset(HW, Ag, P) + (size_t)HW * (C + 4)) * sizeof(float),
                     (hipStream_t)stream, k);
  return scae_launch_status();
}

extern "C" int scae_capsule_head_conv_fwd_tc_f32(
    const float *x, const float *w, const float *bias, int C, float *y, const float *noise_u,
    float noise_scale, int similarity, float *pooled, float *pose, float *presence,
    float *feature, float *absence, int B, int HW, int A, int P, const float *logits,
    const float *w1, const float *b1, const float *w2, const float *b2, float *raw,
    float *templates, float *color, int Ct, int hw, int F, int H1, int template_nonlin,
    int color_nonlin, void *stream) {
  PoolArgs k{};
  k.cx = x, k.cw = w, k.cb = bias, k.cy = y, k.C = C;
  k.out = pooled, k.B = B, k.HW = HW, k.A = A, k.P = P;
  k.splits = pool_splits(B, A);
  k.noise_u = noise_u, k.noise_scale = noise_scale, k.similarity = similarity;
  k.pose = pose, k.presence = presence, k.feature = feature, k.absence = absence;
  int rc = check(k);
  if (rc) return rc;
  if (!scae_capsule_head_conv_supported(HW, A, P, C)) return SCAE_ERR_UNSUPPORTED;
  SCAE_REQUIRE(x && w && y && pooled && pose && presence && feature);
  SCAE_REQUIRE((((size_t)x | (size_t)w) & 15) == 0);
  scae_tc::TcArgs tk{};
  tk.logits = logits, tk.feature = feature, tk.w1 = w1, tk.b1 = b1, tk.w2 = w2, tk.b2 = b2;
  tk.raw = raw, tk.templates = templates, tk.color = color;
  tk.B = B, tk.M = A, tk.C = Ct, tk.hw = hw, tk.F = F, tk.H1 = H1;
  tk.tnl = template_nonlin, tk.cnl = color_nonlin;
  tk.splits = scae_tc::tc_splits(B, A);
  rc = scae_tc::check(tk);
  if (rc) return rc;
  SCAE_REQUIRE(logits && w1 && b1 && w2 && b2 && raw && templates && color);
  if (tk.splits != k.splits || F != P - 8 || k.splits == 1) return SCAE_ERR_UNSUPPORTED;
  const int Ag = A / k.splits;
  const size_t lp = conv_x_offset(HW, Ag, P) + (size_t)HW * (C + 4),
               lt = scae_tc::lds_floats(Ag, Ct, F, H1, false);
  scae::launch(pool_tc_fwd_kernel, dim3(B * k.splits), dim3(NT),
                     (lp > lt ? lp : lt) * sizeof(float), (hipStream_t)stream, k, tk);
  return scae_launch_status();
}

extern "C" int scae_capsule_head_bwd_f32(const float *y, const float *pooled,
                                         const float *noise_u, float noise_scale, int similarity,
                                         const float *g_pose, const float *g_presence,
                                         const float *g_feature, const float *g_feature2,
                                         float *dy, int B, int HW, int A, int P, void *stream) {
  PoolArgs k{};
  k.y = y, k.dy = dy, k.B = B, k.HW = HW, k.A = A, k.P = P;
  k.splits = pool_splits(B, A);
  k.noise_u = noise_u, k.noise_scale = noise_scale, k.similarity = similarity;
  k.pooled = pooled, k.g_pose = g_pose, k.g_presence = g_presence, k.g_feature = g_feature;
  k.g_feature2 = g_feature2;
  int rc = check(k);
  if (rc) return rc;
  if (P < 8) return SCAE_ERR_UNSUPPORTED;
  SCAE_REQUIRE(y && pooled && dy);
  scae::launch(pool_bwd_kernel, dim3(B * k.splits), dim3(NT),
                     lds_floats(HW, A / k.splits, P, true) * sizeof(float),
                     (hipStream_t)stream, k);
  return scae_launch_status();
}
```

torch_scae_amd/ops.py:

```python
import collections
import ctypes
import functools

import numpy as np
import torch

from . import _lib, step_plan
from ._lib import DecoderDesc, ScaeHipError
from .step_plan import StepPlan, current as _plan

__all__ = ["geometric_transform", "qkv_attention", "set_encoder", "grouped_mlp", "seed_attention", "seed_attention_supported", "seed_fold", "seed_fold_supported", "loss_tail", "loss_tail_scalar", "loss_tail_supported", "capsule_votes",
           "capsule_likelihood", "colored_templates", "template_color_supported", "attention_conv_pool", "attention_pool_supported", "capsule_head", "part_encoder", "conv_stack", "conv_stack_supported",
           "uniform", "reset_noise", "pack_params", "render_templates", "render_gmm_log_prob", "render_gmm_log_prob_sums",
           "gmm_log_prob", "gmm_mean", "gmm_mode", "render_gmm_mode", "render_gmm_parts", "GmmParts", "image_sheet", "ScaeHipError"]


def _need_hip(*tensors):
    for t in tensors:
        if t is None:
            continue
        if not t.is_cuda:
            raise ScaeHipError(
                "torch_scae_amd ops run only on a HIP device (got a "
                f"{t.device} tensor); there is no CPU path.")
# ... 831 lines not shown
            and all(k == 3 for k in kernel_sizes)
            and all(s in (1, 2) for s in strides)
            and all(c % 64 == 0 for c in out_channels)
            and all(c <= 1024 for c in chans))


_CONV_RESIDENT_MAX_TILES = 768


def _conv_resident(B, ih, iw, ci, co, s):
    oh, ow = (ih - 3) // s + 1, (iw - 3) // s + 1
    tiles = -(-B * oh * ow // 32) * (co // 64)
    return tiles < _CONV_RESIDENT_MAX_TILES and bool(
        _lib.load().scae_conv3x3_fwd_res_supported(B, ih, iw, ci, co, s))


def _conv_stack_fwd(image, strides, weights, biases, post_bias=None):
    L = len(strides)
    B, C0, H, W = image.shape
    dev, st = image.device, _stream(image)
    new = lambda *shape: torch.empty(*shape, device=dev, dtype=image.dtype)
    c1, s = weights[0].shape[0], strides[0]
    oh, ow = (H - 3) // s + 1, (W - 3) // s + 1
    pro, launch = _plan().prologue, True
    key = lambda ts: [(t.data_ptr(), tuple(t.shape)) for t in ts]
    resident = _conv_bf16_resident(B, oh, ow, weights, strides)
    halves = None
    if pro is not None and pro.first_outs is not None and \
            key([image, *weights, *biases]) == key(
                [pro.first_inputs[0], *pro.first_inputs[1],
                 *pro.first_inputs[2]]) and \
            tuple(strides) == pro.first_inputs[3] and \
            (pro.first_half is not None) == resident:
        act, wfs, wds = pro.first_outs
        halves = pro.first_half
        launch = not pro.first_fresh
    else:
        act = new(B, oh, ow, c1) if not resident else new(1)
        wds, wfs = [], []
        for l in range(1, L):
            co, ci = weights[l].shape[0], weights[l].shape[1]
            wfs.append(new(3, co, 9, ci))
            wds.append(new(ci, 9, co))
        if resident:
            half = lambda *shape: torch.empty(*shape, device=dev,
                                              dtype=torch.bfloat16)
            halves = (half(B, oh, ow, c1),
                      [half(w.shape[0], 9, w.shape[1]) for w in weights[1:]],
                      [half(w.shape[1], 9, w.shape[0]) for w in weights[1:]])
        if pro is not None:
            pro.first_inputs = (image, list(weights), list(biases),
                                tuple(strides))
            pro.first_outs = (act, wfs, wds)
            pro.first_half = halves
    if pro is not None:
        pro.first_fresh = False
    acts = [act]
    n = L - 1
    if launch:
        arr = lambda ts: (ctypes.c_void_p * max(n, 1))(
            *[t.data_ptr() for t in ts])
        ints = lambda v: (ctypes.c_int * max(n, 1))(*v)
        if resident:
            _lib.call("scae_conv3x3_first_fwd_relayout_bf16", _p(image),
                      _p(weights[0]), _p(biases[0]), _p(halves[0]), B, C0, H, W,
                      c1, s, n, arr(weights[1:]), arr(wfs), arr(wds),
                      arr(halves[1]), arr(halves[2]),
                      ints([w.shape[0] for w in weights[1:]]),
                      ints([w.shape[1] for w in weights[1:]]), st)
        else:
            _lib.call("scae_conv3x3_first_fwd_relayout_f32", _p(image),
                      _p(weights[0]), _p(biases[0]), _p(act), B, C0, H, W, c1, s,
                      n, arr(weights[1:]), arr(wfs), arr(wds),
                      ints([w.shape[0] for w in weights[1:]]),
                      ints([w.shape[1] for w in weights[1:]]), st)
    x_post = None
    if resident:
        return _conv_stack_fwd_bf16r(halves, weights, biases, strides,
                                     post_bias, image.dtype)
    for l in range(1, L):
        w, s = weights[l], strides[l]
        co, ci = w.shape[0], w.shape[1]
        ih, iw = act.shape[1], act.shape[2]
        out = new(B, (ih - 3) // s + 1, (iw - 3) // s + 1, co)
        if l == L - 1 and post_bias is not None:
            x_post = torch.empty_like(out)
        conv = (_p(act), _p(wfs[l - 1]), _p(biases[l]), _p(out),
                _p(post_bias if x_post is not None else None), _p(x_post), B,
                ih, iw, ci, co, s)
        carried = False
        if l == 1 and pro is not None and pro.fold_outs is not None:
            if _bf16() or pro.fold_conv_ok is False:
                pro.fold_rides_conv = False
            elif pro.fold_fresh:
                pro.fold_rides_conv = True
            else:
                rc = _lib.load().scae_conv3x3_fwd_fold_f32(
                    *conv, ctypes.byref(_fold_desc(
                        pro.fold_inputs, pro.fold_outs, *pro.fold_dims)), st)
                if rc == _lib.ERR_UNSUPPORTED:
                    pro.fold_conv_ok = pro.fold_rides_conv = False
                else:
                    _lib.check(rc, "scae_conv3x3_fwd_fold_f32")
                    carried = pro.fold_fresh = pro.fold_rides_conv = True
        if not carried:
            if not _bf16() and _conv_resident(B, ih, iw, ci, co, s):
                _lib.call("scae_conv3x3_fwd_res_f32", _p(act),
                          _p(wfs[l - 1][1]), *conv[2:], 0, st)
            else:
                _lib.call(_prec("scae_conv3x3_fwd_f32"), *conv, st)
        acts.append(out)
        act = out
    return acts, wds, x_post


_CONV_BF16R = __import__("os").environ.get("SCAE_CONV_BF16R", "1") != "0"



def _conv_bf16_resident(B, ih, iw, weights, strides):
    if not (_bf16() and _CONV_BF16R and len(strides) >= 2):
        return False
    lib = _lib.load()
    for l in range(1, len(strides)):
        co, ci, s = weights[l].shape[0], weights[l].shape[1], strides[l]
        if not lib.scae_conv3x3_bf16r_supported(B, ih, iw, ci, co, s):
            return False
        ih, iw = (ih - 3) // s + 1, (iw - 3) // s + 1
    return True


def _cvt_bf16(pairs, ref):
    for k in range(0, len(pairs), 8):
        chunk = pairs[k:k + 8]
        n = len(chunk)
        _lib.call("scae_cvt_bf16_batch", n,
                  (ctypes.c_void_p * n)(*[a.data_ptr() for a, _ in chunk]),
                  (ctypes.c_void_p * n)(*[b.data_ptr() for _, b in chunk]),
                  (ctypes.c_int64 * n)(*[a.numel() for a, _ in chunk]),
                  _stream(ref))


def _conv_stack_fwd_bf16r(halves, weights, biases, strides, post_bias, dt):
    act_h, wfh, wdh = halves
    L = len(strides)
    B, dev, st = act_h.shape[0], act_h.device, _stream(act_h)
    half = lambda *shape: torch.empty(*shape, device=dev, dtype=torch.bfloat16)
    acts, x_post = [act_h], None
    for l in range(1, L):
        co, ci, s = weights[l].shape[0], weights[l].shape[1], strides[l]
        ih, iw = act_h.shape[1], act_h.shape[2]
        oh, ow = (ih - 3) // s + 1, (iw - 3) // s + 1
        out_h = half(B, oh, ow, co)
        last = l == L - 1
        out_f = torch.empty(B, oh, ow, co, device=dev, dtype=dt) \
            if last else None
        if last and post_bias is not None:
            x_post = torch.empty_like(out_f)
        _lib.call("scae_conv3x3_fwd_bf16r", _p(act_h), _p(wfh[l - 1]),
                  _p(biases[l]), _p(out_h), _p(out_f),
                  _p(post_bias if x_post is not None else None), _p(x_post),
                  B, ih, iw, ci, co, s, st)
        acts.append(out_f if last else out_h)
        act_h = out_h
    return acts, wdh, x_post


def _conv_stack_bwd(image, acts, wds, strides, wshapes, dpre, gout,
                    defer=False):
    L = len(strides)
    B, C0, H, W = image.shape
    dev, dt, st = image.device, image.dtype, _stream(image)
    new = lambda *shape: torch.empty(*shape, device=dev, dtype=dt)
    gws, gbs = [None] * L, [None] * L
    pending = []
    lib, plan = _lib.load(), _plan()
    resident = L >= 2 and acts[0].dtype == torch.bfloat16
    if resident:
        dpre_h = torch.empty(dpre.shape, device=dev, dtype=torch.bfloat16)
        _cvt_bf16([(dpre.contiguous(), dpre_h)], image)
    for l in (range(L - 1, 0, -1) if resident else ()):
        co, ci = wshapes[l][0], wshapes[l][1]
        xin, s = acts[l - 1], strides[l]
        ih, iw, oh, ow = xin.shape[1], xin.shape[2], dpre_h.shape[1], dpre_h.shape[2]
        splits = lib.scae_conv3x3_wgrad_bf16r_splits(B, oh, ow, ci, co)
        partial = new(splits * (9 * co * ci + co))
        gw, gb = gout(l), gout(L + l)
        _lib.call("scae_conv3x3_wgrad_bf16r", _p(dpre_h), _p(xin), _p(partial),
                  B, ih, iw, ci, co, s, st)
        din_h = torch.empty(B, ih, iw, ci, device=dev, dtype=torch.bfloat16) \
            if l > 1 else None
        din_f = new(B, ih, iw, ci) if l == 1 else None
        _lib.call("scae_conv3x3_dgrad_bf16r", _p(dpre_h), _p(wds[l - 1]),
                  _p(xin), _p(din_h), _p(din_f), B, ih, iw, ci, co, s, st)
        pending.append((partial, gw, gb, co, ci, splits))
        gws[l], gbs[l] = gw, gb
        dpre_h = din_h
        dpre = din_f
    for l in (range(L - 1, 0, -1) if not resident else ()):
        co, ci = wshapes[l][0], wshapes[l][1]
        xin, s = acts[l - 1], strides[l]
        ih, iw, oh, ow = xin.shape[1], xin.shape[2], dpre.shape[1], dpre.shape[2]
        splits = _lib.load().scae_conv3x3_wgrad_splits(B, oh, ow, ci, co)
        partial = new(splits * (9 * co * ci + co))
        gw, gb = gout(l), gout(L + l)
        din = new(B, ih, iw, ci)
        pair = (_p(dpre), _p(wds[l - 1]), _p(xin), _p(din), _p(partial), B, ih,
                iw, ci, co, s)
        carried = False
        if not plan.bf16 and l <= 2:
            parked = plan.take("reduce")
            if parked is not None:
                rc = lib.scae_conv3x3_bwd_pair_reduce_f32(
                    *pair, *parked.args, st) if l == 2 else _lib.ERR_UNSUPPORTED
                if rc == _lib.ERR_UNSUPPORTED:
                    parked.launch_alone()
                else:
                    _lib.check(rc, "scae_conv3x3_bwd_pair_reduce_f32")
                    carried = True
            parked = None if carried or l != 1 else plan.take("fold_bwd")
            if parked is not None:
                rc = lib.scae_conv3x3_bwd_pair_fold_f32(
                    *pair, ctypes.byref(parked.desc),
                    ctypes.byref(parked.grads), st)
                if rc == _lib.ERR_UNSUPPORTED:
                    parked.launch_alone()
                else:
                    _lib.check(rc, "scae_conv3x3_bwd_pair_fold_f32")
                    carried = True
        if not carried:
            _lib.call(_prec("scae_conv3x3_bwd_pair_f32"), *pair, st)
        pending.append((partial, gw, gb, co, ci, splits))
        gws[l], gbs[l] = gw, gb
        dpre = din
    c1 = wshapes[0][0]
    k1 = C0 * 9 + 1
    partial = new(_lib.load().scae_conv3x3_first_wgrad_rows(B, c1), c1, k1)
    n = len(pending)
    arr = lambda k: (ctypes.c_void_p * max(n, 1))(
        *[p[k].data_ptr() for p in pending])
    ints = lambda k: (ctypes.c_int * max(n, 1))(*[p[k] for p in pending])
    _lib.call("scae_conv3x3_first_wgrad_reduce_f32", _p(dpre), _p(image),
              _p(partial), B, C0, H, W, c1, strides[0], n, arr(0), arr(1),
              arr(2), ints(3), ints(4), ints(5), st)
    gws[0], gbs[0] = _sum_rows(partial.view(partial.shape[0], -1),
                               [(c1, C0, 3, 3), (c1,)],
                               outs=[gout(0), gout(L)], defer=defer)
    return gws, gbs


class _ConvStack(torch.autograd.Function):

    @_fwd
    def forward(ctx, image, strides, *wb):
        _need_hip(image, *wb)
        L = len(strides)
        image = image.contiguous()
        weights = [w.contiguous() for w in wb[:L]]
        biases = [b.contiguous() for b in wb[L:]]
        acts, wds, _ = _conv_stack_fwd(image, strides, weights, biases)
        ctx.save_for_backward(image, *acts, *wds)
        ctx.meta = (tuple(strides), [tuple(w.shape) for w in weights])
        ctx.slots = [_slot(t, ctx) for t in wb]
        ctx.refs = [tuple(t.shape) for t in wb]
        return acts[-1].permute(0, 3, 1, 2)

    @_bwd
    def backward(ctx, gy):
        strides, wshapes = ctx.meta
        L = len(strides)
        image = ctx.saved_tensors[0]
        acts = ctx.saved_tensors[1:1 + L]
        wds = ctx.saved_tensors[1 + L:]
        dpre = torch.ops.aten.threshold_backward(
            gy.permute(0, 2, 3, 1).contiguous(), acts[-1], 0.0)
        gws, gbs = _conv_stack_bwd(
            image, acts, wds, strides, wshapes, dpre,
            lambda i: _grad_out(ctx.slots[i], image, ctx.refs[i]))
        return (None, None, *gws, *gbs)


def conv_stack(image, weights, biases, strides):
    return _ConvStack.apply(image, tuple(int(s) for s in strides), *weights,
                            *biases)


def attention_pool_supported(HW, A, P):
    return bool(_lib.load().scae_attention_pool_supported(HW, A, P))


_CONV1X1_KMAX = int(__import__("os").environ.get("SCAE_CONV1X1_KMAX", "1024"))


def _conv1x1_fwd(x, weight, bias):
    B, HW, C = x.shape
    AP = weight.shape[0]
    y = torch.empty(B, HW, AP, device=x.device, dtype=x.dtype)
    _gemm(_p(x), _p(weight), _p(y), 1, B * HW, AP, C, True, C, 0, True, C, 0,
          AP, 0, bias=_p(bias), bias_ld=1, ref=x)
    return y


def _conv1x1_bwd(x, weight, dy, gate=None, outs=None, raw_sum=None,
                 defer=False):
    B, HW, C = x.shape
    AP = weight.shape[0]
    gsz = max(d for d in range(1, B + 1)
              if B % d == 0 and (d == 1 or HW * d <= _CONV1X1_KMAX))
    S, kper, slab = B // gsz, HW * gsz, AP * C + AP
    part = torch.empty(S, slab, device=x.device, dtype=x.dtype)
    dx = torch.empty_like(x)
    dgrad = _gemm_desc(_p(dy), _p(weight), _p(dx), 1, B * HW, C, AP, True, AP,
                       0, False, C, 0, C, 0)
    raw = None
    if gate is not None:
        raw = torch.empty_like(x)
        dgrad.mask, dgrad.ldmask, dgrad.c_nomask = gate.data_ptr(), C, \
            raw.data_ptr()
    _gemm_pair(
        _gemm_desc(_p(dy), _p(x), _p(part), S, AP, C, kper, False, AP,
                   kper * AP, False, C, kper * C, C, slab,
                   asum=_off(part, AP * C), asum_b=slab), dgrad, x)
    jobs = [dict(partial=part, shapes=[tuple(weight.shape), (AP,)], outs=outs,
                 defer=defer)]
    if raw_sum is not None:
        jobs.append(dict(partial=raw.view(B, HW * C), shapes=[raw_sum[0]],
                         transpose=C, outs=[raw_sum[1]], defer=defer))
    gw, gb = _sum_rows_multi(jobs)[0]
    return (dx, gw, gb) if gate is None else (dx, gw, gb, raw)


class _AttentionConvPool(torch.autograd.Function):

    @_fwd
    def forward(ctx, x, weight, bias, n_caps):
        _need_hip(x, weight, bias)
        x, weight, bias = x.contiguous(), weight.contiguous(), bias.contiguous()
        B, HW, C = x.shape
        P = weight.shape[0] // n_caps
        y = _conv1x1_fwd(x, weight, bias)
        out = torch.empty(B, n_caps, P - 1, device=x.device, dtype=x.dtype)
        _lib.call("scae_attention_pool_fwd_f32", _p(y), _p(out), B, HW, n_caps,
                  P, _stream(x))
        ctx.save_for_backward(x, weight, y)
        ctx.n_caps = n_caps
        return out

    @_bwd
    def backward(ctx, g):
        x, weight, y = ctx.saved_tensors
        B, HW, C = x.shape
        A = ctx.n_caps
        dy = torch.empty_like(y)
        _lib.call("scae_attention_pool_bwd_f32", _p(y), _p(g.contiguous()),
                  _p(dy), B, HW, A, weight.shape[0] // A, _stream(x))
        return (*_conv1x1_bwd(x, weight, dy), None)


def _capsule_head_fwd(x, weight, bias, noise_u, n_caps, noise_scale,
                      similarity):
    B, HW, C = x.shape
    P = weight.shape[0] // n_caps
    F = P - 8
    new = lambda *shape: torch.empty(*shape, device=x.device, dtype=x.dtype)
    pooled, pose, presence = new(B, n_caps, P - 1), new(B, n_caps, 6), \
        new(B, n_caps)
    feature = new(B, n_caps, F) if F > 0 else None
    absence = new(B, n_caps, 1)
    head = (_p(noise_u), float(noise_scale), int(similarity), _p(pooled),
            _p(pose), _p(presence), _p(feature), _p(absence), B, HW, n_caps, P,
            _stream(x))
    if _lib.load().scae_capsule_head_conv_preferred(B, HW, n_caps, P, C) and \
            (x.data_ptr() | weight.data_ptr()) % 16 == 0:
        y = new(B, HW, n_caps * P)
        offer = _plan().offers.get("tc_fwd")
        if offer is not None and feature is not None and offer.result is None \
                and offer.M == n_caps and offer.F == F and offer.ok:
            raw = new(1, n_caps, offer.C, *offer.hw)
            templates = new(B, n_caps, offer.C, *offer.hw)
            color = new(B, n_caps, offer.C)
            if _lib.try_call(
                    "scae_capsule_head_conv_fwd_tc_f32", _p(x), _p(weight),
                    _p(bias), C, _p(y), *head[:-1],
                    *[_p(t) for t in offer.params], _p(raw), _p(templates),
                    _p(color), offer.C, offer.hw[0] * offer.hw[1], F, offer.H1,
                    *offer.codes, head[-1]):
                offer.result, offer.feature = (raw, templates, color), feature
                return y, pooled, pose, presence, feature, absence
            offer.ok = False
        _lib.call("scae_capsule_head_conv_fwd_f32", _p(x), _p(weight),
                  _p(bias), C, _p(y), *head)
    else:
        y = _conv1x1_fwd(x, weight, bias)
        _lib.call("scae_capsule_head_fwd_f32", _p(y), *head)
    return y, pooled, pose, presence, feature, absence


class _CapsuleHead(torch.autograd.Function):

    @_fwd
    def forward(ctx, x, weight, bias, noise_u, n_caps, noise_scale, similarity):
        _need_hip(x, weight, bias, noise_u)
        x, weight, bias = x.contiguous(), weight.contiguous(), bias.contiguous()
        noise_u = _c(noise_u)
        B, HW, C = x.shape
        P = weight.shape[0] // n_caps
        F = P - 8
        new = lambda *shape: torch.empty(*shape, device=x.device, dtype=x.dtype)
        y, pooled, pose, presence, feature, absence = _capsule_head_fwd(
            x, weight, bias, noise_u, n_caps, noise_scale, similarity)
        ctx.save_for_backward(x, weight, y, pooled,
                              *([noise_u] if noise_u is not None else []))
        ctx.meta = (n_caps, float(noise_scale), int(similarity),
                    noise_u is not None)
        ctx.set_materialize_grads(False)
        if feature is None:
            feature = new(B, n_caps, 0)
            ctx.mark_non_differentiable(feature)
        ctx.mark_non_differentiable(absence)
        return pose, presence, feature, absence

    @_bwd
    def backward(ctx, g_pose, g_presence, g_feature, _g_absence):
        x, weight, y, pooled = ctx.saved_tensors[:4]
        A, noise_scale, similarity, has_noise = ctx.meta
        noise_u = ctx.saved_tensors[4] if has_noise else None
        B, HW, C = x.shape
        dy = torch.empty_like(y)
        _lib.call("scae_capsule_head_bwd_f32", _p(y), _p(pooled), _p(noise_u),
                  noise_scale, similarity, _p(_c(g_pose)), _p(_c(g_presence)),
                  _p(_c(g_feature)), None, _p(dy), B, HW, A,
                  weight.shape[0] // A, _stream(x))
        return (*_conv1x1_bwd(x, weight, dy), None, None, None, None)


def capsule_head(x, weight, bias, n_caps, noise_u=None, noise_scale=0.,
                 similarity=False):
    pose, presence, feature, absence = _CapsuleHead.apply(
        x, weight, bias, noise_u, n_caps, noise_scale, similarity)
    return pose, presence, (feature if feature.shape[-1] > 0 else None), absence


class _PartEncoder(torch.autograd.Function):

    @_fwd
    def forward(ctx, image, strides, post_bias, att_w, att_b, noise_u, n_caps,
                noise_scale, similarity, *wb):
        _need_hip(image, post_bias, att_w, att_b, noise_u, *wb)
        L = len(strides)
        image = image.contiguous()
        weights = [w.contiguous() for w in wb[:L]]
        biases = [b.contiguous() for b in wb[L:]]
        acts, wds, x = _conv_stack_fwd(image, strides, weights, biases,
                                       post_bias.contiguous())
        B, OH, OW, C = x.shape
        HW = OH * OW
        x = x.view(B, HW, C)
        att_w2 = att_w.contiguous().view(-1, C)
        P = att_w2.shape[0] // n_caps
        F = P - 8
        noise_u = _c(noise_u)
        new = lambda *shape: torch.empty(*shape, device=x.device, dtype=x.dtype)
        y, pooled, pose, presence, feature, absence = _capsule_head_fwd(
            x, att_w2, att_b.contiguous(), noise_u, n_caps, noise_scale,
            similarity)
        ctx.save_for_backward(image, *acts, *wds, x, att_w2, y, pooled,
                              *([noise_u] if noise_u is not None else []))
        ctx.meta = (tuple(strides), [tuple(w.shape) for w in weights], n_caps,
                    float(noise_scale), int(similarity), noise_u is not None,
                    tuple(post_bias.shape), tuple(att_w.shape))
        ctx.slots = [_slot(t, ctx) for t in (post_bias, att_w, att_b, *wb)]
        ctx.refs = [tuple(t.shape) for t in wb]
        ctx.set_materialize_grads(False)
        if feature is None:
            feature = new(B, n_caps, 0)
            ctx.mark_non_differentiable(feature)
        twin = torch.empty(0, device=x.device, dtype=x.dtype).set_(
            feature.untyped_storage(), feature.storage_offset(),
            feature.shape, feature.stride())
        if F <= 0:
            ctx.mark_non_differentiable(twin)
        ctx.mark_non_differentiable(absence)
        return pose, presence, feature, twin, absence

    @_bwd
    def backward(ctx, g_pose, g_presence, g_feature, g_twin, _g_absence):
        (strides, wshapes, A, noise_scale, similarity, has_noise, pb_shape,
         attw_shape) = ctx.meta
        L = len(strides)
        saved = ctx.saved_tensors
        image, acts, wds = saved[0], saved[1:1 + L], saved[1 + L:2 * L]
        x, att_w2, y, pooled = saved[2 * L:2 * L + 4]
        noise_u = saved[2 * L + 4] if has_noise else None
        B, HW, C = x.shape
        dy = torch.empty_like(y)
        P_ = att_w2.shape[0] // A
        head = (_p(y), _p(pooled), _p(noise_u), noise_scale, similarity,
                _p(_c(g_pose)), _p(_c(g_presence)))
        parked, carried = ctx.plan.take("tc_bwd"), False
        if parked is not None:
            mine = [t for t in (g_twin, g_feature) if t is not None
                    and t.is_contiguous() and t.data_ptr() == parked.gf_ptr]
            rc = _lib.ERR_UNSUPPORTED
            if len(mine) == 1 and parked.bm == (B, A):
                other = g_feature if mine[0] is g_twin else g_twin
                rc = _lib.load().scae_capsule_head_bwd_tc_f32(
                    *head, _p(_c(other)), _p(dy), B, HW, A, P_, *parked.ptrs,
                    *parked.dims, _stream(x))
            if rc == _lib.ERR_UNSUPPORTED:
                parked.launch_alone()
            else:
                _lib.check(rc, "scae_capsule_head_bwd_tc_f32")
                carried = True
        if not carried:
            _lib.call("scae_capsule_head_bwd_f32", *head, _p(_c(g_feature)),
                      _p(_c(g_twin)), _p(dy), B, HW, A, P_, _stream(x))
        act = acts[-1]
        g_attw = _grad_out(ctx.slots[1], x, attw_shape)
        g_attb = _grad_out(ctx.slots[2], x, (att_w2.shape[0],))
        g_pb = _grad_out(ctx.slots[0], x, pb_shape)
        dpre, _, _, _ = _conv1x1_bwd(x, att_w2, dy, gate=act.view(B, HW, C),
                                     outs=[g_attw, g_attb],
                                     raw_sum=(pb_shape, g_pb),
                                     defer=all(sl is not None
                                               for sl in ctx.slots[:3]))
        gws, gbs = _conv_stack_bwd(
            image, acts, wds, strides, wshapes, dpre.view(act.shape),
            lambda i: _grad_out(ctx.slots[3 + i], image, ctx.refs[i]),
            defer=ctx.slots[3] is not None and ctx.slots[3 + L] is not None)
        return (None, None, g_pb, g_attw, g_attb, None, None, None, None,
                *gws, *gbs)


def part_encoder(image, weights, biases, strides, post_bias, att_weight,
                 att_bias, n_caps, noise_u=None, noise_scale=0.,
                 similarity=False):
    pose, presence, feature, twin, absence = _PartEncoder.apply(
        image, tuple(int(s) for s in strides), post_bias, att_weight, att_bias,
        noise_u, n_caps, noise_scale, similarity, *weights, *biases)
    if feature.shape[-1] == 0:
        feature = twin = None
    return pose, presence, feature, twin, absence


def attention_conv_pool(x, weight, bias, n_caps):
    return _AttentionConvPool.apply(x, weight, bias, n_caps)


class _PendingClassProbs:

    def __init__(self, args, keep, stream_ref):
        self.args, self.keep, self.ref = args, keep, stream_ref

    def launch_alone(self):
        _lib.call("scae_class_probs_f32", *self.args, _stream(self.ref))


class _PendingCombine:

    def __init__(self, tail_args, keep, loss_ptr, out_ptr, stream_ref):
        self.tail, self.keep, self.ref = tail_args, keep, stream_ref
        self.loss_ptr, self.out_ptr = loss_ptr, out_ptr

    def launch_alone(self):
        ex = self.keep[-1]
        ex.defer_combine = 0
        _lib.call("scae_loss_tail_combine_f32", *self.tail, _stream(self.ref))


def flush_pending_forward():
    _plan().flush_scope("fusing")


def class_probs_supported(O, ncls):
    return bool(_lib.load().scae_class_probs_supported(O, ncls))


class _ClassProbs(torch.autograd.Function):

    @_fwd
    def forward(ctx, caps_presence, posterior, weight, bias, extra_sums):
        _need_hip(caps_presence, posterior, weight, bias)
        cp, post = caps_presence.detach().contiguous(), \
            posterior.detach().contiguous()
        weight, bias = weight.contiguous(), bias.contiguous()
        B, O1, M = post.shape
        ncls = weight.shape[0]
        prior = torch.empty(B, ncls, device=cp.device, dtype=cp.dtype)
        posterior_prob = torch.empty_like(prior)
        extra = list(extra_sums or ())
        args = (_p(cp), _p(post), _p(weight), _p(bias), _p(prior),
                _p(posterior_prob), B, O1 - 1, M, ncls, _sum_jobs(extra),
                len(extra))
        if ctx.plan.fused:
            ctx.plan.flush_scope("fusing")
            ctx.plan.park("class_probs", _PendingClassProbs(
                args, (cp, post, weight, bias, prior, posterior_prob, extra),
                cp))
        else:
            _lib.call("scae_class_probs_f32", *args, _stream(cp))
        ctx.save_for_backward(cp, post, weight, bias)
        ctx.set_materialize_grads(False)
        return prior, posterior_prob

    @_bwd
    def backward(ctx, g_prior, g_post):
        cp, post, weight, bias = ctx.saved_tensors
        with torch.enable_grad():
            w, b = weight.detach().requires_grad_(), bias.detach().requires_grad_()
            outs, gs = [], []
            for x, g in ((cp, g_prior), (post[:, :-1].sum(-1), g_post)):
                if g is not None:
                    outs.append(torch.softmax(
                        torch.nn.functional.linear(x, w, b), -1))
                    gs.append(g)
            gw, gb = torch.autograd.grad(outs, (w, b), gs) if outs else (None,
                                                                         None)
        return None, None, gw, gb, None


def class_probs(caps_presence, posterior, weight, bias, extra_sums=None):
    return _ClassProbs.apply(caps_presence, posterior, weight, bias, extra_sums)


_NONLIN_CODE = {"sigmoid": 0, "relu1": 1}


def template_color_supported(M, C, F, H1, template_nonlin, color_nonlin):
    return (template_nonlin in _NONLIN_CODE and color_nonlin in _NONLIN_CODE
            and bool(_lib.load().scae_template_color_supported(M, C, F, H1)))


class _TcOffer:

    def __init__(self, logits, w1, b1, w2, b2, tnl, cnl):
        _need_hip(logits, w1, b1, w2, b2)
        self.params = [t.detach().contiguous() for t in (logits, w1, b1, w2, b2)]
        _, self.M, self.C, th, tw = logits.shape
        self.hw, self.F, self.H1 = (th, tw), w1.shape[1], w1.shape[0]
        self.codes = (tnl, cnl)
        self.result = self.feature = None
        self.ok = True

    def serves(self, logits, feature, w1, b1, w2, b2, tnl, cnl):
        return self.result is not None and self.codes == (tnl, cnl) and \
            self.feature.data_ptr() == feature.data_ptr() and \
            self.feature.shape == feature.shape and all(
                a.data_ptr() == b.data_ptr() and a.shape == b.shape
                for a, b in zip(self.params, (logits, w1, b1, w2, b2)))


def offer_colored_templates(template_logits, w1, b1, w2, b2, template_nonlin,
                            color_nonlin):
    plan = _plan()
    if plan.fused and (torch.is_grad_enabled() or plan.evaluation is not None) \
            and template_logits.is_cuda:
        plan.offer("tc_fwd", _TcOffer(template_logits, w1, b1, w2, b2,
                                      _NONLIN_CODE[template_nonlin],
                                      _NONLIN_CODE[color_nonlin]))


def withdraw_colored_templates_offer():
    _plan().claim("tc_fwd")


class _ColoredTemplates(torch.autograd.Function):
    @_fwd
    def forward(ctx, logits, feature, w1, b1, w2, b2, tnl, cnl,
                feature_node=None):
        _need_hip(logits, feature, w1, b1, w2, b2)
        logits, feature, w1, b1, w2, b2 = (t.contiguous() for t in (
            logits, feature, w1, b1, w2, b2))
        _, M, C, th, tw = logits.shape
        B, F, H1 = feature.shape[0], feature.shape[2], w1.shape[0]
        new = lambda *shape: torch.empty(*shape, device=logits.device,
                                         dtype=logits.dtype)
        offer = ctx.plan.claim("tc_fwd")
        if offer is not None and offer.serves(logits, feature, w1, b1, w2, b2,
                                              tnl, cnl):
            raw, templates, color = offer.result
        else:
            raw, templates, color = new(1, M, C, th, tw), \
                new(B, M, C, th, tw), new(B, M, C)
            _lib.call("scae_template_color_fwd_f32", _p(logits), _p(feature),
                      _p(w1), _p(b1), _p(w2), _p(b2), _p(raw), _p(templates),
                      _p(color), B, M, C, th * tw, F, H1, tnl, cnl,
                      _stream(logits))
        ctx.save_for_backward(logits, feature, w1, b1, w2, b2, color)
        ctx.codes = (tnl, cnl)
        ctx.slots = [_slot(t, ctx) for t in (logits, w1, b1, w2, b2)]
        ctx.set_materialize_grads(False)
        ctx.feature_node = feature_node
        return raw, templates

    @_bwd
    def backward(ctx, g_raw, g_templates):
        logits, feature, w1, b1, w2, b2, color = ctx.saved_tensors
        _, M, C, th, tw = logits.shape
        B, F, H1 = feature.shape[0], feature.shape[2], w1.shape[0]
        if g_templates is None:
            g_templates = torch.zeros(B, M, C, th, tw, device=logits.device,
                                      dtype=logits.dtype)
        n1, n2, n3 = H1 * F, H1 * F + H1, H1 * F + H1 + C * H1
        g_logits = _grad_out(ctx.slots[0], logits)
        g_feature = torch.empty_like(feature)
        rows = _lib.load().scae_template_color_partial_rows(B, M)
        partial = torch.empty(rows, n3 + C, device=logits.device,
                              dtype=logits.dtype)
        g_templates, g_raw = g_templates.contiguous(), _c(g_raw)
        ptrs = (_p(logits), _p(feature), _p(w1), _p(b1), _p(w2), _p(b2),
                _p(color), _p(g_templates), _p(g_raw), _p(g_logits),
                _p(g_feature), _p(partial))
        dims = (C, th * tw, F, H1, *ctx.codes)
        outs = [_grad_out(sl, t) for sl, t in zip(ctx.slots[1:],
                                                  (w1, b1, w2, b2))]
        if ctx.plan.parking and ctx.feature_node == "_PartEncoderBackward" \
                and _in_slot(g_logits) and all(_in_slot(o) for o in outs):
            ctx.plan.park("tc_bwd", _PendingTcBackward(
                ptrs, (B, M), dims, (logits, feature, w1, b1, w2, b2, color,
                                     g_templates, g_raw, partial),
                g_feature.data_ptr(), logits))
        else:
            _lib.call("scae_template_color_bwd_f32", *ptrs, B, M, *dims,
                      _stream(logits))
        gw1, gb1, gw2, gb2 = _sum_rows(
            partial, [(H1, F), (H1,), (C, H1), (C,)], outs=outs,
            defer=all(sl is not None for sl in ctx.slots[1:5]))
        return g_logits, g_feature, gw1, gb1, gw2, gb2, None, None, None


def colored_templates(template_logits, feature, w1, b1, w2, b2,
                      template_nonlin, color_nonlin):
    node = type(feature.grad_fn).__name__ if feature.grad_fn is not None \
        else None
    return _ColoredTemplates.apply(template_logits, feature, w1, b1, w2, b2,
                                   _NONLIN_CODE[template_nonlin],
                                   _NONLIN_CODE[color_nonlin], node)


def _gemm(A, B, C, batch, M, N, K, a_k, lda, a_b, b_k, ldb, b_b, ldc, c_b,
          bias=None, bias_ld=1, bias_b=0, mask=None, ldmask=0, mask_b=0,
          relu=False, asum=None, asum_b=0, asum_ld=1, ref=None):
    _lib.call(_prec("scae_gemm_f32"), A, B, C, bias, mask, asum, batch, M, N, K,
              int(a_k), lda, a_b, int(b_k), ldb, b_b, ldc, c_b, bias_ld, bias_b,
              ldmask, mask_b, asum_b, asum_ld, int(relu), _stream(ref))


def _gemm_desc(A, B, C, batch, M, N, K, a_k, lda, a_b, b_k, ldb, b_b, ldc, c_b,
               bias=None, bias_ld=1, bias_b=0, mask=None, ldmask=0, mask_b=0,
               relu=False, asum=None, asum_b=0, asum_ld=1):
    d = _lib.GemmDesc()
    for name, ptr in (("A", A), ("B", B), ("C", C), ("bias", bias),
                      ("mask", mask), ("asum", asum)):
        setattr(d, name, None if ptr is None else ptr.value)
    d.batch, d.M, d.N, d.K = batch, M, N, K
    d.a_kcontig, d.lda, d.a_batch = int(a_k), lda, a_b
    d.b_kcontig, d.ldb, d.b_batch = int(b_k), ldb, b_b
    d.ldc, d.c_batch = ldc, c_b
    d.bias_ld, d.bias_batch = bias_ld, bias_b
    d.ldmask, d.mask_batch, d.asum_batch, d.relu = ldmask, mask_b, asum_b, \
        int(relu)
    d.asum_ld = asum_ld
    return d


def _gemm_pair(first, second, ref):
    _lib.call(_prec("scae_gemm_pair_f32"), ctypes.byref(first), ctypes.byref(second),
              _stream(ref))


def _off(t, nfloats=0):
    return ctypes.c_void_p(t.data_ptr() + 4 * nfloats)


class _GroupedMLP(torch.autograd.Function):

    @_fwd
    def forward(ctx, x, ones_input, n_layers, grad_pregated, x_is_relu,
                pad_out, *wb):
        _need_hip(x, *wb)
        if x.stride(2) != 1:
            x = x.contiguous()
        weights = [w.contiguous() for w in wb[:n_layers]]
        biases = [None if b is None else b.contiguous() for b in wb[n_layers:]]
        B, G, Kin = x.shape
        if ones_input and biases[0] is not None:
            raise ScaeHipError("ones_input with a bias is not built")
        acts = []
        cur, cur_ld, cur_b, K = x, x.stride(0), x.stride(1), Kin
        for l, (w, b) in enumerate(zip(weights, biases)):
            N, ldb = w.shape[1], w.shape[2]
            last = l == n_layers - 1
            if last:
                Np = (N + 3) // 4 * 4 if pad_out else N
                out = torch.empty(B, G, Np, device=x.device,
                                  dtype=x.dtype)[:, :, :N]
                ldc, c_b = G * Np, Np
            else:
                out = torch.empty(G, B, N, device=x.device, dtype=x.dtype)
                ldc, c_b = N, B * N
            if l == 0 and ones_input:
                bias, bias_ld, bias_b = _off(w, Kin), ldb, N * ldb
            elif b is not None:
                bias, bias_ld, bias_b = _p(b), 1, N
            else:
                bias, bias_ld, bias_b = None, 1, 0
            _gemm(_p(cur), _p(w), _p(out), G, B, N, K, True, cur_ld, cur_b, True,
                  ldb, N * ldb, ldc, c_b, bias, bias_ld, bias_b, relu=True,
                  ref=x)
            acts.append(out)
            cur, cur_ld, cur_b, K = out, N, B * N, N
        ctx.save_for_backward(x, *weights, *acts)
        ctx.meta = (bool(ones_input), n_layers,
                    [b is not None for b in biases], bool(grad_pregated),
                    bool(x_is_relu))
        ctx.slots = [_slot(t, ctx) for t in wb]
        return acts[-1]

    @_bwd
    def backward(ctx, gy):
        ones_input, L, has_bias, pregated, x_is_relu = ctx.meta
        x = ctx.saved_tensors[0]
        weights = ctx.saved_tensors[1:1 + L]
        acts = ctx.saved_tensors[1 + L:]
        B, G, Kin = x.shape
        dev, dt = x.device, x.dtype
        gpre = gy
        if not pregated:
# ... 1479 lines not shown
```

torch_scae_amd/step_plan.py:

```python
import collections
import contextlib
import contextvars
import weakref

ANY = "*"
_LIVE = weakref.WeakSet()


class Ride:

    __slots__ = ("carriers", "readers", "scope", "abi", "what")

    def __init__(self, what, carriers, readers=(), scope="deferring", abi=""):
        self.what, self.carriers, self.readers = what, tuple(carriers), readers
        self.scope, self.abi = scope, abi


RIDES = collections.OrderedDict([
    ("tc_fwd", Ride(
        "the colour MLP's forward (K10)",
        carriers=("_PartEncoder.forward",), scope="offer",
        abi="scae_capsule_head_conv_fwd_tc_f32")),
    ("logprob_fwd", Ride(
        "the reconstruction likelihood's forward (K1)",
        carriers=("_SetEncoder.forward",), scope="offer",
        abi="scae_set_encoder_fwd_logprob_f32")),
    ("class_probs", Ride(
        "SCAE.forward's two classifier heads (one wave per image)",
        carriers=("_LossTail.forward",), scope="fusing",
        abi="scae_loss_tail_fwd_class_probs_f32")),
    ("combine", Ride(
        "the loss tail's batch combine (one workgroup)",
        carriers=("_LossTail.backward",), scope="fusing",
        abi="scae_loss_tail_bwd_f32 (scae_loss_extras.defer_combine)")),
    ("k1_bwd", Ride(
        "the reconstruction likelihood's backward (K1)",
        carriers=("_CapsuleLikelihood.backward",), readers=ANY,
        abi="scae_render_gmm_sums_bwd_likelihood_f32")),
    ("wgrads", Ride(
        "the capsule MLPs' four weight-gradient GEMMs",
        carriers=("_SeedAttention.backward",),
        abi="scae_seed_attention_mfma_bwd_gemm_f32")),
    ("tc_bwd", Ride(
        "the colour MLP's backward (K10)",
        carriers=("_PartEncoder.backward",),
        readers=("_CapsuleHead.backward",),
        abi="scae_capsule_head_bwd_tc_f32")),
    ("reduce", Ride(
        "the output attention's partial-row reduction",
        carriers=("_PartEncoder.backward", "_ConvStack.backward"),
        abi="scae_conv3x3_bwd_pair_reduce_f32")),
    ("fold_bwd", Ride(
        "the folding products' backward (K2d)",
        carriers=("_PartEncoder.backward", "_ConvStack.backward"),
        abi="scae_conv3x3_bwd_pair_fold_f32")),
])


class StepPlan:
    def __init__(self, name="step", prologue=None):
        _LIVE.add(self)
        self.name = name
        self.target = None
        self.rider = None
        self.offers = {}
        self.parked = {}
        self.deferred = None
        self.sums_to_optimizer = False
        self.held_sums = []
        self.prologue = prologue
        self.bf16 = False
        self.noise = {}
        self.noise_salt = 0
        self.side_stream = None
        self.evaluation = None
        self.train_log = None

    @contextlib.contextmanager
    def active(self):
        token = _CURRENT.set(self)
        try:
            yield self
        finally:
            _CURRENT.reset(token)

    @property
    def fused(self):
        return self.target is not None

    @property
    def parking(self):
        return self.target is not None and self.deferred is not None

    def offer(self, kind, work):
        assert RIDES[kind].scope == "offer", kind
        self.offers[kind] = work

    def claim(self, kind):
        return self.offers.pop(kind, None)

    def park(self, kind, work):
        assert kind in RIDES and RIDES[kind].scope != "offer", kind
        stale = self.parked.pop(kind, None)
        if stale is not None:
            stale.launch_alone()
        self.parked[kind] = work

    def take(self, kind):
        return self.parked.pop(kind, None)

    def holds(self, kind, work=None):
        held = self.parked.get(kind)
        return held is not None and (work is None or held is work)

    def flush(self, *kinds):
        for kind in RIDES:
            if (not kinds or kind in kinds) and kind in self.parked:
                self.parked.pop(kind).launch_alone()

    def flush_scope(self, scope):
        self.flush(*[k for k, r in RIDES.items() if r.scope == scope])

    def enter(self, node):
        if not self.parked:
            return
        for kind in RIDES:
            if kind not in self.parked:
                continue
            ride = RIDES[kind]
            if node in ride.carriers:
                continue
            if ride.readers == ANY or node in ride.readers:
                self.parked.pop(kind).launch_alone()

    def flush_sums(self):
        if self.deferred:
            units = list(self.deferred)
            del self.deferred[:]
            from . import ops
            ops._launch_sum_units(units)

    def take_held_sums(self):
        units, self.held_sums = self.held_sums, []
        return units

    @contextlib.contextmanager
    def fusing(self, target):
        prev = (self.target, self.rider)
        self.target, self.rider = target, None
        self.parked.clear()
        self.offers.clear()
        ok = False
        try:
            yield self
            ok = True
        finally:
            self.target, self.rider = prev
            self.offers.clear()
            if ok:
                self.flush_scope("fusing")

    @contextlib.contextmanager
    def deferring(self):
        outer = self.deferred
        if outer is None:
            self.deferred = []
        ok = False
        try:
            yield self
            ok = True
        finally:
            if outer is None:
                try:
                    if ok:
                        self.flush_scope("deferring")
                        if self.sums_to_optimizer:
                            self.held_sums.extend(self.deferred)
                            del self.deferred[:]
                        else:
                            self.flush_sums()
                finally:
                    self.deferred = None

    @contextlib.contextmanager
    def with_prologue(self, pro):
        prev, self.prologue = self.prologue, pro
        try:
            yield pro
        finally:
            self.prologue = prev

    @contextlib.contextmanager
    def evaluating(self, epilogue):
        prev, self.evaluation = self.evaluation, epilogue
        try:
            yield self
        finally:
            self.evaluation = prev

    @contextlib.contextmanager
    def logging(self, train_log):
        prev, self.train_log = self.train_log, train_log
        try:
            yield self
        finally:
            self.train_log = prev

    @contextlib.contextmanager
    def precision(self, bf16):
        prev, self.bf16 = self.bf16, bool(bf16)
        try:
            yield self
        finally:
            self.bf16 = prev


def live_plans():
    return list(_LIVE)


_CURRENT = contextvars.ContextVar("scae_step_plan", default=None)
ambient = StepPlan("ambient")


def current():
    plan = _CURRENT.get()
    return ambient if plan is None else plan


@contextlib.contextmanager
def running(plan, node):
    token = _CURRENT.set(plan)
    try:
        plan.enter(node)
        yield plan
    finally:
        _CURRENT.reset(token)
```

Baseline: 261,300.

## Add pooled capsule head that projects attention-pooled features instead of full conv output

```diff
diff --git a/include/scae_hip.h b/include/scae_hip.h
--- a/include/scae_hip.h
+++ b/include/scae_hip.h
@@ -356,6 +356,40 @@
     const float *g_templates, const float *g_raw, float *g_logits, float *tc_g_feature,
     float *partial, int C, int hw, int F, int H1, int template_nonlin, int color_nonlin,
     void *stream);
+
+int scae_capsule_head_pooled_preferred(int B, int HW, int A, int P, int C);
+int scae_capsule_head_pooled_fwd_f32(const float *x, const float *w, const float *bias, int C,
+                                     float *m, float *xm, const float *noise_u,
+                                     float noise_scale, int similarity, float *pooled,
+                                     float *pose, float *presence, float *feature,
+                                     float *absence, int B, int HW, int A, int P, int images,
+                                     void *stream);
+int scae_capsule_head_pooled_fwd_tc_f32(
+    const float *x, const float *w, const float *bias, int C, float *m, float *xm,
+    const float *noise_u, float noise_scale, int similarity, float *pooled, float *pose,
+    float *presence, float *feature, float *absence, int B, int HW, int A, int P, int images,
+    const float *logits, const float *w1, const float *b1, const float *w2, const float *b2,
+    float *raw, float *templates, float *color, int Ct, int hw, int F, int H1,
+    int template_nonlin, int color_nonlin, void *stream);
+int scae_capsule_head_pooled_bwd_f32(
+    const float *x, const float *w, const float *bias, int C, const float *m,
+    const float *pooled, const float *noise_u, float noise_scale, int similarity,
+    const float *g_pose, const float *g_presence, const float *g_feature,
+    const float *g_feature2, float *gs, float *v, float *dl, float *xdl, float *brow, int B,
+    int HW, int A, int P, void *stream);
+int scae_capsule_head_pooled_bwd_tc_f32(
+    const float *x, const float *w, const float *bias, int C, const float *m,
+    const float *pooled, const float *noise_u, float noise_scale, int similarity,
+    const float *g_pose, const float *g_presence, const float *g_feature, float *gs, float *v,
+    float *dl, float *xdl, float *brow, int B, int HW, int A, int P, const float *logits,
+    const float *feature, const float *w1, const float *b1, const float *w2, const float *b2,
+    const float *color, const float *g_templates, const float *g_raw, float *g_logits,
+    float *tc_g_feature, float *partial, int Ct, int hw, int F, int H1, int template_nonlin,
+    int color_nonlin, void *stream);
+int scae_capsule_head_pooled_grads_f32(
+    const float *w, const float *m, const float *xm, const float *gs, const float *v,
+    const float *dl, const float *xdl, const float *brow, const float *gate, float *dx,
+    float *raw, float *part, int B, int HW, int A, int P, int C, int S, void *stream);
 
 int scae_rmsprop_step_f32(float *param, const float *grad, float *square_avg, float *buf,
                           int64_t n, float lr, const float *lr_dev, float alpha, float eps,
diff --git a/torch_scae_amd/_lib.py b/torch_scae_amd/_lib.py
--- a/torch_scae_amd/_lib.py
+++ b/torch_scae_amd/_lib.py
@@ -325,6 +325,16 @@
     "scae_capsule_head_bwd_f32": [P, P, P, c_float, c_int, P, P, P, P, P] + [c_int] * 4 + [P],
     "scae_capsule_head_bwd_tc_f32": [P, P, P, c_float, c_int, P, P, P, P] + [c_int] * 4
     + [P] * 12 + [c_int] * 6 + [P],
+    "scae_capsule_head_pooled_preferred": [c_int] * 5,
+    "scae_capsule_head_pooled_fwd_f32": [P, P, P, c_int, P, P, P, c_float, c_int, P, P, P, P, P]
+    + [c_int] * 5 + [P],
+    "scae_capsule_head_pooled_fwd_tc_f32": [P, P, P, c_int, P, P, P, c_float, c_int, P, P, P,
+                                            P, P] + [c_int] * 5 + [P] * 8 + [c_int] * 6 + [P],
+    "scae_capsule_head_pooled_bwd_f32": [P, P, P, c_int, P, P, P, c_float, c_int] + [P] * 9
+    + [c_int] * 4 + [P],
+    "scae_capsule_head_pooled_bwd_tc_f32": [P, P, P, c_int, P, P, P, c_float, c_int] + [P] * 8
+    + [c_int] * 4 + [P] * 12 + [c_int] * 6 + [P],
+    "scae_capsule_head_pooled_grads_f32": [P] * 12 + [c_int] * 6 + [P],
     "scae_template_color_supported": [c_int] * 4,
     "scae_template_color_partial_rows": [c_int] * 2,
     "scae_template_color_fwd_f32": [P] * 9 + [c_int] * 8 + [P],
diff --git a/torch_scae_amd/csrc/attention_pool.hip b/torch_scae_amd/csrc/attention_pool.hip
--- a/torch_scae_amd/csrc/attention_pool.hip
+++ b/torch_scae_amd/csrc/attention_pool.hip
@@ -139,6 +139,30 @@
   }
 }
 
+__device__ __forceinline__ void head_outputs(const PoolArgs &k, const float *pooled, size_t cap0,
+                                             int A) {
+  const int P = k.P, F = P - 8;
+  for (int a = threadIdx.x; a < A; a += NT) {
+    const float *row = pooled + a * (P - 1);
+    scae_gt::GtState st;
+    scae_gt::gt_eval(row, 1, st);
+    float o[6];
+    scae_gt::gt_rows(st, k.similarity, o);
+#pragma unroll
+    for (int j = 0; j < 6; ++j) k.pose[(cap0 + a) * 6 + j] = o[j];
+    float logit = row[6];
+    if (k.noise_u) logit += (k.noise_u[cap0 + a] - .5f) * k.noise_scale;
+    const float pr = scae::sigmoidf_(logit);
+    k.presence[cap0 + a] = pr;
+    if (k.absence) k.absence[cap0 + a] = 1.f - pr;
+  }
+  if (k.feature)
+    for (int e = threadIdx.x; e < A * F; e += NT) {
+      const int a = e / F, f = e - a * F;
+      k.feature[cap0 * F + e] = pooled[a * (P - 1) + 7 + f];
+    }
+}
+
 __device__ __forceinline__ void pool_fwd_body(const PoolArgs &k, float *lds, int blk) {
   const int Af = k.A, A = Af / k.splits, b = blk / k.splits, a0 = (blk % k.splits) * A;
   const int HW = k.HW, P = k.P, AP = A * P, APp = padded(AP), ldy = Af * P;
@@ -167,26 +191,7 @@
   }
   if (!k.pose) return;
   __syncthreads();
-  const int F = P - 8;
-  for (int a = threadIdx.x; a < A; a += NT) {
-    const float *row = pooled + a * (P - 1);
-    scae_gt::GtState st;
-    scae_gt::gt_eval(row, 1, st);
-    float o[6];
-    scae_gt::gt_rows(st, k.similarity, o);
-#pragma unroll
-    for (int j = 0; j < 6; ++j) k.pose[(cap0 + a) * 6 + j] = o[j];
-    float logit = row[6];
-    if (k.noise_u) logit += (k.noise_u[cap0 + a] - .5f) * k.noise_scale;
-    const float pr = scae::sigmoidf_(logit);
-    k.presence[cap0 + a] = pr;
-    if (k.absence) k.absence[cap0 + a] = 1.f - pr;
-  }
-  if (k.feature)
-    for (int e = threadIdx.x; e < A * F; e += NT) {
-      const int a = e / F, f = e - a * F;
-      k.feature[cap0 * F + e] = pooled[a * (P - 1) + 7 + f];
-    }
+  head_outputs(k, pooled, cap0, A);
 }
 __global__ __launch_bounds__(NT) void pool_fwd_kernel(PoolArgs k) {
   extern __shared__ __align__(16) float lds[];
@@ -199,6 +204,33 @@
   __threadfence_block();
   __syncthreads();
   scae_tc::tc_fwd_body<NT>(tk, lds, blockIdx.x);
+}
+
+__device__ __forceinline__ void head_grad_rows(const PoolArgs &k, float *gs, size_t cap0, int A) {
+  const int P = k.P, F = P - 8;
+  for (int a = threadIdx.x; a < A; a += NT) {
+    const float *row = k.pooled + (cap0 + a) * (P - 1);
+    float raw[6], go[6], gp[6];
+#pragma unroll
+    for (int j = 0; j < 6; ++j) {
+      raw[j] = row[j];
+      go[j] = k.g_pose ? k.g_pose[(cap0 + a) * 6 + j] : 0.f;
+    }
+    scae_gt::GtState st;
+    scae_gt::gt_eval(raw, 1, st);
+    scae_gt::gt_backward(st, k.similarity, go, gp);
+#pragma unroll
+    for (int j = 0; j < 6; ++j) gs[a * (P - 1) + j] = gp[j];
+    float logit = row[6];
+    if (k.noise_u) logit += (k.noise_u[cap0 + a] - .5f) * k.noise_scale;
+    const float sg = scae::sigmoidf_(logit);
+    gs[a * (P - 1) + 6] = k.g_presence ? k.g_presence[cap0 + a] * sg * (1.f - sg) : 0.f;
+  }
+  for (int e = threadIdx.x; e < A * F; e += NT) {
+    const int a = e / F, f = e - a * F;
+    gs[a * (P - 1) + 7 + f] = (k.g_feature ? k.g_feature[cap0 * F + e] : 0.f) +
+                              (k.g_feature2 ? k.g_feature2[cap0 * F + e] : 0.f);
+  }
 }
 
 __device__ __forceinline__ void pool_bwd_body(const PoolArgs &k, float *lds, int blk) {
@@ -209,30 +241,7 @@
         *sa = gs + A * (P - 1);
   stage_y(ys, k.y + (size_t)b * HW * ldy + a0 * P, HW, AP, APp, ldy);
   if (k.pooled) {
-    const int F = P - 8;
-    for (int a = threadIdx.x; a < A; a += NT) {
-      const float *row = k.pooled + (cap0 + a) * (P - 1);
-      float raw[6], go[6], gp[6];
-#pragma unroll
-      for (int j = 0; j < 6; ++j) {
-        raw[j] = row[j];
-        go[j] = k.g_pose ? k.g_pose[(cap0 + a) * 6 + j] : 0.f;
-      }
-      scae_gt::GtState st;
-      scae_gt::gt_eval(raw, 1, st);
-      scae_gt::gt_backward(st, k.similarity, go, gp);
-#pragma unroll
-      for (int j = 0; j < 6; ++j) gs[a * (P - 1) + j] = gp[j];
-      float logit = row[6];
-      if (k.noise_u) logit += (k.noise_u[cap0 + a] - .5f) * k.noise_scale;
-      const float sg = scae::sigmoidf_(logit);
-      gs[a * (P - 1) + 6] = k.g_presence ? k.g_presence[cap0 + a] * sg * (1.f - sg) : 0.f;
-    }
-    for (int e = threadIdx.x; e < A * F; e += NT) {
-      const int a = e / F, f = e - a * F;
-      gs[a * (P - 1) + 7 + f] = (k.g_feature ? k.g_feature[cap0 * F + e] : 0.f) +
-                                (k.g_feature2 ? k.g_feature2[cap0 * F + e] : 0.f);
-    }
+    head_grad_rows(k, gs, cap0, A);
   } else {
     for (int e = threadIdx.x; e < A * (P - 1); e += NT) gs[e] = k.g[cap0 * (P - 1) + e];
   }
@@ -277,6 +286,489 @@
   scae_tc::tc_bwdA_body<NT>(tk, lds, blockIdx.x);
   __syncthreads();
   pool_bwd_body(k, lds, blockIdx.x);
+}
+
+struct PooledArgs {
+  PoolArgs k;
+  float *m, *xm;
+  int G;
+  float *gs, *v, *dl;
+  float *xdl;
+  float *brow;
+};
+
+struct PooledFwdLds {
+  int xs, xms, ls, mask, msum, pooled, total, LS;
+};
+__host__ __device__ inline PooledFwdLds pooled_fwd_lds(int G, int HW, int A, int P, int C) {
+  PooledFwdLds l;
+  l.LS = (G * A) | 1;
+  l.xs = 0;
+  l.xms = G * HW * (C + 4);
+  l.ls = l.xms + G * A * C;
+  l.mask = l.ls + HW * l.LS;
+  l.msum = l.mask + G * A * HW;
+  l.pooled = l.msum + G * A;
+  l.total = l.pooled + G * A * (P - 1);
+  return l;
+}
+
+template <int CTRL>
+__device__ __forceinline__ double dpp_d(double v) {
+  const int lo = __builtin_amdgcn_update_dpp(0, __double2loint(v), CTRL, 0xf, 0xf, true);
+  const int hi = __builtin_amdgcn_update_dpp(0, __double2hiint(v), CTRL, 0xf, 0xf, true);
+  return __hiloint2double(hi, lo);
+}
+__device__ __forceinline__ double row_sum16_d(double v) {
+  v += dpp_d<0xB1>(v);
+  v += dpp_d<0x4E>(v);
+  v += dpp_d<0x141>(v);
+  v += dpp_d<0x140>(v);
+  return v;
+}
+
+template <int NB>
+__device__ __forceinline__ double dot_lane(const float4 (&w)[NB], const float *row, int l) {
+  double s = 0.;
+#pragma unroll
+  for (int t = 0; t < NB; ++t) {
+    const float4 r = scae_wave::ld4(row + 64 * t + 4 * l);
+    s = fma((double)w[t].x, (double)r.x, s), s = fma((double)w[t].y, (double)r.y, s);
+    s = fma((double)w[t].z, (double)r.z, s), s = fma((double)w[t].w, (double)r.w, s);
+  }
+  return s;
+}
+
+template <int NB>
+__device__ __forceinline__ void stage_x_rows(float *xs, const float *x, int rows) {
+  constexpr int C = 64 * NB, XS = C + 4, q4 = C / 4;
+  for (int base = 0; base < rows * q4; base += 2 * NT) {
+    const int e0 = base + threadIdx.x, e1 = e0 + NT;
+    const int r0 = e0 / q4, c0 = 4 * (e0 - r0 * q4), r1 = e1 / q4, c1 = 4 * (e1 - r1 * q4);
+    float4 v0, v1;
+    if (e0 < rows * q4) v0 = scae_wave::ld4(x + (size_t)r0 * C + c0);
+    if (e1 < rows * q4) v1 = scae_wave::ld4(x + (size_t)r1 * C + c1);
+    if (e0 < rows * q4) *reinterpret_cast<float4 *>(xs + r0 * XS + c0) = v0;
+    if (e1 < rows * q4) *reinterpret_cast<float4 *>(xs + r1 * XS + c1) = v1;
+  }
+}
+
+template <int NB>
+__device__ __forceinline__ int pooled_fwd_body(const PooledArgs &h, float *lds, int blk) {
+  using namespace scae_wave;
+  const PoolArgs &k = h.k;
+  constexpr int C = 64 * NB, XS = C + 4;
+  const int Af = k.A, A = Af / k.splits, a0 = (blk % k.splits) * A, b0 = (blk / k.splits) * h.G;
+  const int nb = min(h.G, k.B - b0), HW = k.HW, P = k.P, GA = nb * A;
+  const PooledFwdLds o = pooled_fwd_lds(h.G, HW, A, P, C);
+  float *xs = lds + o.xs, *xms = lds + o.xms, *ls = lds + o.ls, *mask = lds + o.mask,
+        *msum = lds + o.msum, *pooled = lds + o.pooled;
+  const int lane = threadIdx.x & 63, wave = threadIdx.x >> 6, r = lane & 15, q = lane >> 4;
+  const int ncol = (A + 15) / 16, nrow = (HW + 15) / 16, units = nb * ncol * nrow;
+  float4 wf[4 * NB];
+  float lbias = 0.f;
+  auto load_w = [&](int col) {
+    const int ca = min(col * 16 + r, A - 1);
+    const float *wr = k.cw + ((size_t)(a0 + ca) * P + P - 1) * C + 4 * q;
+#pragma unroll
+    for (int t = 0; t < 4 * NB; ++t) wf[t] = ld4(wr + 16 * t);
+    lbias = k.cb ? k.cb[(a0 + ca) * P + P - 1] : 0.f;
+  };
+  if (wave < units) load_w((wave / nrow) % ncol);
+  stage_x_rows<NB>(xs, k.cx + (size_t)b0 * HW * C, nb * HW);
+  __syncthreads();
+  for (int u = wave; u < units; u += NT / 64) {
+    const int rt = u % nrow, col = (u / nrow) % ncol, g = u / (nrow * ncol);
+    if (u != wave) load_w(col);
+    const int ca = col * 16 + r;
+    const float bias = lbias;
+    const int pix = rt * 16 + r;
+    const float *xr = xs + (g * HW + (pix < HW ? pix : HW - 1)) * XS + 4 * q;
+    f32x4 acc = splat(0.f);
+#pragma unroll
+    for (int t = 0; t < 4 * NB; ++t) acc = mma16(acc, ld4(xr + 16 * t), wf[t]);
+    if (ca < A) {
+#pragma unroll
+      for (int j = 0; j < 4; ++j) {
+        const int p = rt * 16 + 4 * q + j;
+        if (p < HW) ls[p * o.LS + g * A + ca] = acc[j] + bias;
+      }
+    }
+  }
+  __syncthreads();
+  constexpr int PRE = NB <= 2 ? 6 : 3;
+  const int l = threadIdx.x & 15, rows = A * (P - 1);
+  float4 pw[PRE][NB];
+  float pb[PRE];
+  auto load_row = [&](int row, float4 (&w)[NB], float &bias) {
+    const int ca = row / (P - 1), p = row - ca * (P - 1);
+    const float *wr = k.cw + ((size_t)(a0 + ca) * P + p) * C;
+#pragma unroll
+    for (int t = 0; t < NB; ++t) w[t] = ld4(wr + 64 * t + 4 * l);
+    bias = k.cb ? k.cb[(a0 + ca) * P + p] : 0.f;
+  };
+#pragma unroll
+  for (int i = 0; i < PRE; ++i) {
+    const int row = (threadIdx.x >> 4) + i * (NT / 16);
+    if (row < rows) load_row(row, pw[i], pb[i]);
+  }
+  softmax_masks(mask, ls, HW, GA, 1, o.LS);
+  __syncthreads();
+  for (int e = threadIdx.x; e < GA * HW; e += NT) {
+    const int ga = e / HW, g = ga / A, ca = ga - g * A;
+    h.m[((size_t)(b0 + g) * Af + a0 + ca) * HW + (e - ga * HW)] = mask[e];
+  }
+  for (int ga = threadIdx.x; ga < GA; ga += NT) {
+    float s = 0.f;
+    for (int i = 0; i < HW; ++i) s += mask[ga * HW + i];
+    msum[ga] = s;
+  }
+  for (int e = threadIdx.x; e < GA * C; e += NT) {
+    const int ga = e / C, c = e - ga * C, g = ga / A, ca = ga - g * A;
+    const float *xc = xs + g * HW * XS + c;
+    double d = 0.;
+    for (int i = 0; i < HW; ++i) d = fma((double)mask[ga * HW + i], (double)xc[i * XS], d);
+    const float s = (float)d;
+    xms[e] = s;
+    h.xm[((size_t)(b0 + g) * Af + a0 + ca) * C + c] = s;
+  }
+  __syncthreads();
+  auto project = [&](int row, const float4 (&w)[NB], float bias) {
+    const int ca = row / (P - 1), p = row - ca * (P - 1);
+    for (int g = 0; g < nb; ++g) {
+      const int ga = g * A + ca;
+      const double s = row_sum16_d(dot_lane<NB>(w, xms + ga * C, l));
+      if (l == 0) {
+        const float val = (float)fma((double)bias, (double)msum[ga], s);
+        pooled[ga * (P - 1) + p] = val;
+        k.out[((size_t)(b0 + g) * Af + a0 + ca) * (P - 1) + p] = val;
+      }
+    }
+  };
+#pragma unroll
+  for (int i = 0; i < PRE; ++i) {
+    const int row = (threadIdx.x >> 4) + i * (NT / 16);
+    if (row < rows) project(row, pw[i], pb[i]);
+  }
+  for (int row = (threadIdx.x >> 4) + PRE * (NT / 16); row < rows; row += NT / 16) {
+    float4 w[NB];
+    float bias;
+    load_row(row, w, bias);
+    project(row, w, bias);
+  }
+  __syncthreads();
+  for (int g = 0; g < nb; ++g)
+    head_outputs(k, pooled + g * A * (P - 1), (size_t)(b0 + g) * Af + a0, A);
+  return nb;
+}
+__device__ __forceinline__ int pooled_fwd_any(const PooledArgs &h, float *lds, int blk) {
+  switch (h.k.C / 64) {
+    case 1: return pooled_fwd_body<1>(h, lds, blk);
+    case 2: return pooled_fwd_body<2>(h, lds, blk);
+    case 3: return pooled_fwd_body<3>(h, lds, blk);
+    default: return pooled_fwd_body<4>(h, lds, blk);
+  }
+}
+__global__ __launch_bounds__(NT) void pooled_fwd_kernel(PooledArgs h) {
+  extern __shared__ __align__(16) float lds[];
+  pooled_fwd_any(h, lds, blockIdx.x);
+}
+__global__ __launch_bounds__(NT) void pooled_tc_fwd_kernel(PooledArgs h, scae_tc::TcArgs tk) {
+  extern __shared__ __align__(16) float lds[];
+  const int nb = pooled_fwd_any(h, lds, blockIdx.x);
+  const int grp = blockIdx.x % h.k.splits, b0 = (blockIdx.x / h.k.splits) * h.G;
+  for (int g = 0; g < nb; ++g) {
+    __threadfence_block();
+    __syncthreads();
+    scae_tc::tc_fwd_body<NT>(tk, lds, (b0 + g) * h.k.splits + grp);
+  }
+}
+
+struct PooledBwdLds {
+  int xs, vs, vpart, gs, mask, dls, msum, td, total, SL;
+};
+__host__ __device__ inline PooledBwdLds pooled_bwd_lds(int HW, int A, int P, int C) {
+  PooledBwdLds l;
+  const int pairs = A * C / 4;
+  l.SL = pairs >= NT ? 1 : (NT / pairs < 4 ? NT / pairs : 4);
+  l.xs = 0;
+  l.vs = HW * (C + 4);
+  l.vpart = l.vs + A * C;
+  l.gs = l.vpart + l.SL * A * C;
+  l.mask = l.gs + A * (P - 1);
+  l.dls = l.mask + A * HW;
+  l.msum = l.dls + A * HW;
+  l.td = (l.msum + A + 1) & ~1;
+  l.total = l.td + 2 * (A * HW + A);
+  return l;
+}
+template <int NB>
+__device__ __forceinline__ void pooled_bwd_body(const PooledArgs &h, float *lds, int blk) {
+  using namespace scae_wave;
+  const PoolArgs &k = h.k;
+  constexpr int C = 64 * NB, XS = C + 4, q4 = C / 4;
+  const int Af = k.A, A = Af / k.splits, b = blk / k.splits, a0 = (blk % k.splits) * A;
+  const int HW = k.HW, P = k.P;
+  const size_t cap0 = (size_t)b * Af + a0;
+  const PooledBwdLds o = pooled_bwd_lds(HW, A, P, C);
+  float *xs = lds + o.xs, *vs = lds + o.vs, *vpart = lds + o.vpart, *gs = lds + o.gs,
+        *mask = lds + o.mask, *dls = lds + o.dls, *msum = lds + o.msum;
+  double *td = reinterpret_cast<double *>(lds + o.td), *sad = td + A * HW;
+  constexpr int VB = 12;
+  const int pairs = A * q4, per = (P - 1 + o.SL - 1) / o.SL;
+  auto v_item = [&](int u, int &a, int &c, int &pb, int &pe) {
+    const int sl = u / pairs, pr = u - sl * pairs;
+    a = pr / q4, c = 4 * (pr - a * q4);
+    pb = sl * per, pe = min(P - 1, (sl + 1) * per);
+    return sl;
+  };
+  float4 wv[VB];
+  if ((int)threadIdx.x < pairs * o.SL) {
+    int a, c, pb, pe;
+    v_item(threadIdx.x, a, c, pb, pe);
+    const float *wc = k.cw + (size_t)(a0 + a) * P * C + c;
+#pragma unroll
+    for (int j = 0; j < VB; ++j)
+      if (pb + j < pe) wv[j] = ld4(wc + (size_t)(pb + j) * C);
+  }
+  head_grad_rows(k, gs, cap0, A);
+  stage_x_rows<NB>(xs, k.cx + (size_t)b * HW * C, HW);
+  for (int e = threadIdx.x; e < A * HW; e += NT) mask[e] = h.m[cap0 * HW + e];
+  __syncthreads();
+  for (int e = threadIdx.x; e < A * (P - 1); e += NT) h.gs[cap0 * (P - 1) + e] = gs[e];
+  for (int u = threadIdx.x; u < pairs * o.SL; u += NT) {
+    int a, c, pb, pe;
+    const int sl = v_item(u, a, c, pb, pe);
+    const float *wc = k.cw + (size_t)(a0 + a) * P * C + c;
+    float4 s = make_float4(0.f, 0.f, 0.f, 0.f);
+    auto add = [&](int p, const float4 &w) {
+      const float g = gs[a * (P - 1) + p];
+      s.x = fmaf(g, w.x, s.x), s.y = fmaf(g, w.y, s.y);
+      s.z = fmaf(g, w.z, s.z), s.w = fmaf(g, w.w, s.w);
+    };
+    int p = pb;
+    if (u == (int)threadIdx.x) {
+#pragma unroll
+      for (int j = 0; j < VB; ++j)
+        if (pb + j < pe) add(pb + j, wv[j]);
+      p = min(pe, pb + VB);
+    }
+#pragma unroll 6
+    for (; p < pe; ++p) add(p, ld4(wc + (size_t)p * C));
+    *reinterpret_cast<float4 *>(vpart + (sl * A + a) * C + c) = s;
+  }
+  for (int a = threadIdx.x; a < A; a += NT) {
+    float sm = 0.f;
+    for (int i = 0; i < HW; ++i) sm += mask[a * HW + i];
+    msum[a] = sm;
+  }
+  __syncthreads();
+  for (int e = threadIdx.x; e < A * C; e += NT) {
+    float s = vpart[e];
+    for (int sl = 1; sl < o.SL; ++sl) s += vpart[sl * A * C + e];
+    vs[e] = s;
+    h.v[cap0 * C + e] = s;
+  }
+  __syncthreads();
+  const int l = threadIdx.x & 15;
+  for (int e = threadIdx.x >> 4; e < A * HW; e += NT / 16) {
+    const int a = e / HW, pix = e - a * HW;
+    double s = 0.;
+#pragma unroll
+    for (int u = 0; u < NB; ++u) {
+      const float4 w = ld4(vs + a * C + 64 * u + 4 * l), r = ld4(xs + pix * XS + 64 * u + 4 * l);
+      s = fma((double)w.x, (double)r.x, s), s = fma((double)w.y, (double)r.y, s);
+      s = fma((double)w.z, (double)r.z, s), s = fma((double)w.w, (double)r.w, s);
+    }
+    s = row_sum16_d(s);
+    if (l == 0) td[e] = s;
+  }
+  __syncthreads();
+  for (int u = threadIdx.x; u < ((A * 32 + NT - 1) / NT) * NT; u += NT) {
+    const int a = u >> 5, l32 = u & 31;
+    double s = 0.;
+    if (a < A)
+      for (int pix = l32; pix < HW; pix += 32) s = fma((double)mask[a * HW + pix], td[a * HW + pix], s);
+    s = row_sum16_d(s);
+    s += __shfl_xor(s, 16, 64);
+    if (a < A && l32 == 0) sad[a] = s;
+  }
+  __syncthreads();
+  for (int e = threadIdx.x; e < A * HW; e += NT) {
+    const float d = (float)((double)mask[e] * (td[e] - sad[e / HW]));
+    dls[e] = d;
+    h.dl[cap0 * HW + e] = d;
+  }
+  __syncthreads();
+  for (int e = threadIdx.x; e < A * C; e += NT) {
+    const int a = e / C, c = e - a * C;
+    float s = 0.f;
+    for (int i = 0; i < HW; ++i) s = fmaf(dls[a * HW + i], xs[i * XS + c], s);
+    h.xdl[cap0 * C + e] = s;
+  }
+  float *brow = h.brow + (size_t)b * Af * P + a0 * P;
+  for (int e = threadIdx.x; e < A * P; e += NT) {
+    const int a = e / P, p = e - a * P;
+    float s;
+    if (p < P - 1)
+      s = gs[a * (P - 1) + p] * msum[a];
+    else {
+      double d = 0.;
+      for (int i = 0; i < HW; ++i) d += (double)dls[a * HW + i];
+      s = (float)d;
+    }
+    brow[e] = s;
+  }
+}
+__device__ __forceinline__ void pooled_bwd_any(const PooledArgs &h, float *lds, int blk) {
+  switch (h.k.C / 64) {
+    case 1: pooled_bwd_body<1>(h, lds, blk); break;
+    case 2: pooled_bwd_body<2>(h, lds, blk); break;
+    case 3: pooled_bwd_body<3>(h, lds, blk); break;
+    default: pooled_bwd_body<4>(h, lds, blk); break;
+  }
+}
+__global__ __launch_bounds__(NT) void pooled_bwd_kernel(PooledArgs h) {
+  extern __shared__ __align__(16) float lds[];
+  pooled_bwd_any(h, lds, blockIdx.x);
+}
+__global__ __launch_bounds__(NT) void pooled_tc_bwd_kernel(PooledArgs h, scae_tc::TcArgs tk,
+                                                           int nA) {
+  extern __shared__ __align__(16) float lds[];
+  if ((int)blockIdx.x >= nA) {
+    scae_tc::tc_bwdB_body<NT>(tk, (int)blockIdx.x - nA);
+    return;
+  }
+  scae_tc::tc_bwdA_body<NT>(tk, lds, blockIdx.x);
+  __syncthreads();
+  pooled_bwd_any(h, lds, blockIdx.x);
+}
+
+struct PooledGradArgs {
+  const float *w, *m, *xm, *gs, *v, *dl, *xdl, *brow, *gate;
+  float *dx, *raw, *part;
+  int B, HW, A, P, C, S, gsz, nW;
+};
+constexpr int GB = 32;
+__host__ __device__ inline size_t pooled_grads_lds(int HW, int A, int P) {
+  const size_t w = (size_t)2 * GB * 64 + (size_t)GB * (2 * P - 1), x = (size_t)2 * A * 64 + (size_t)2 * A * HW;
+  return w > x ? w : x;
+}
+__global__ __launch_bounds__(NT) void pooled_grads_kernel(PooledGradArgs k) {
+  using scae_wave::ld4;
+  extern __shared__ __align__(16) float lds[];
+  const int lane = threadIdx.x & 63, wave = __builtin_amdgcn_readfirstlane(threadIdx.x >> 6);
+  const int HW = k.HW, A = k.A, P = k.P, C = k.C, nch = C / 64;
+  int blk = blockIdx.x;
+  if (blk < k.nW) {
+    const int ch = blk % nch, a = (blk / nch) % A, s = blk / nch / A, c0 = ch * 64;
+    const size_t b0 = (size_t)s * k.gsz;
+    float *xms = lds, *xdls = xms + GB * 64, *gss = xdls + GB * 64, *brs = gss + GB * (P - 1);
+    float *out = k.part + (size_t)s * ((size_t)A * P * C + (size_t)A * P);
+    for (int p0 = 0; p0 < P; p0 += 4 * (NT / 64)) {
+      const bool bias = ch == 0 && p0 == 0;
+      float acc[4] = {0.f, 0.f, 0.f, 0.f};
+      double bsum = 0.;
+      for (int bc = 0; bc < k.gsz; bc += GB) {
+        const int n = min(GB, k.gsz - bc);
+        if (bc || p0) __syncthreads();
+        {
+          const int e = threadIdx.x, r = e >> 4, q = e & 15;
+          const size_t at = ((b0 + bc + r) * A + a) * C + c0 + 4 * q;
+          float4 x4, d4;
+          if (e < n * 16) x4 = ld4(k.xm + at), d4 = ld4(k.xdl + at);
+          const int ng = n * (P - 1), nr = bias ? n * P : 0;
+          for (int base = 0; base < max(ng, nr); base += 2 * NT) {
+            float g[2], br[2];
+#pragma unroll
+            for (int j = 0; j < 2; ++j) {
+              const int f = base + j * NT + threadIdx.x, rg = f / (P - 1), rb = f / P;
+              if (f < ng) g[j] = k.gs[((b0 + bc + rg) * A + a) * (P - 1) + (f - rg * (P - 1))];
+              if (f < nr) br[j] = k.brow[((b0 + bc + rb) * A + a) * P + (f - rb * P)];
+            }
+#pragma unroll
+            for (int j = 0; j < 2; ++j) {
+              const int f = base + j * NT + threadIdx.x;
+              if (f < ng) gss[f] = g[j];
+              if (f < nr) brs[f] = br[j];
+            }
+          }
+          if (e < n * 16) {
+            *reinterpret_cast<float4 *>(xms + r * 64 + 4 * q) = x4;
+            *reinterpret_cast<float4 *>(xdls + r * 64 + 4 * q) = d4;
+          }
+        }
+        __syncthreads();
+        for (int r = 0; r < n; ++r) {
+          const float xv = xms[r * 64 + lane], xd = xdls[r * 64 + lane];
+#pragma unroll
+          for (int j = 0; j < 4; ++j) {
+            const int p = p0 + wave + (NT / 64) * j;
+            if (p < P - 1)
+              acc[j] = fmaf(gss[r * (P - 1) + p], xv, acc[j]);
+            else if (p == P - 1)
+              acc[j] += xd;
+          }
+        }
+        if (bias && (int)threadIdx.x < P)
+          for (int r = 0; r < n; ++r) bsum += (double)brs[r * P + threadIdx.x];
+      }
+#pragma unroll
+      for (int j = 0; j < 4; ++j) {
+        const int p = p0 + wave + (NT / 64) * j;
+        if (p < P) out[((size_t)a * P + p) * C + c0 + lane] = acc[j];
+      }
+      if (bias && (int)threadIdx.x < P) out[(size_t)A * P * C + a * P + threadIdx.x] = (float)bsum;
+    }
+    return;
+  }
+  blk -= k.nW;
+  const int ch = blk % nch, b = blk / nch, c0 = ch * 64;
+  float *vs = lds, *wls = vs + A * 64, *ms = wls + A * 64, *dls = ms + A * HW;
+  for (int base = 0; base < max(A * 16, (A * HW + 1) / 2); base += NT) {
+    const int e = base + threadIdx.x, a = e >> 4, q = e & 15;
+    float4 v4, w4;
+    float mr[2], dr[2];
+    if (e < A * 16) {
+      v4 = ld4(k.v + ((size_t)b * A + a) * C + c0 + 4 * q);
+      w4 = ld4(k.w + ((size_t)a * P + P - 1) * C + c0 + 4 * q);
+    }
+#pragma unroll
+    for (int j = 0; j < 2; ++j) {
+      const int f = 2 * base + j * NT + threadIdx.x;
+      if (f < A * HW) mr[j] = k.m[(size_t)b * A * HW + f], dr[j] = k.dl[(size_t)b * A * HW + f];
+    }
+    if (e < A * 16) {
+      *reinterpret_cast<float4 *>(vs + a * 64 + 4 * q) = v4;
+      *reinterpret_cast<float4 *>(wls + a * 64 + 4 * q) = w4;
+    }
+#pragma unroll
+    for (int j = 0; j < 2; ++j) {
+      const int f = 2 * base + j * NT + threadIdx.x;
+      if (f < A * HW) ms[f] = mr[j], dls[f] = dr[j];
+    }
+  }
+  __syncthreads();
+  double acc[4] = {0., 0., 0., 0.};
+  int pix[4];
+#pragma unroll
+  for (int j = 0; j < 4; ++j) pix[j] = min(wave + (NT / 64) * j, HW - 1);
+  for (int a = 0; a < A; ++a) {
+    const double vv = vs[a * 64 + lane], wl = wls[a * 64 + lane];
+#pragma unroll
+    for (int j = 0; j < 4; ++j)
+      acc[j] = fma((double)ms[a * HW + pix[j]], vv, fma((double)dls[a * HW + pix[j]], wl, acc[j]));
+  }
+#pragma unroll
+  for (int j = 0; j < 4; ++j) {
+    const int i = wave + (NT / 64) * j;
+    if (i < HW) {
+      const size_t at = ((size_t)b * HW + i) * C + c0 + lane;
+      const float d = (float)acc[j];
+      if (k.raw) k.raw[at] = d;
+      k.dx[at] = (!k.gate || k.gate[at] > 0.f) ? d : 0.f;
+    }
+  }
 }
 
 int check(const PoolArgs &k) {
@@ -462,3 +954,179 @@
                      (hipStream_t)stream, k);
   return scae_launch_status();
 }
+
+namespace {
+constexpr size_t kPooledLdsMax = 64 * 1024;
+inline int pooled_images(int, int) { return 1; }
+
+int pooled_fwd_args(PooledArgs &h, const float *x, const float *w, const float *bias, int C,
+                    float *m, float *xm, const float *noise_u, float noise_scale, int similarity,
+                    float *pooled, float *pose, float *presence, float *feature, float *absence,
+                    int B, int HW, int A, int P, int images) {
+  h = PooledArgs{};
+  PoolArgs &k = h.k;
+  k.cx = x, k.cw = w, k.cb = bias, k.C = C;
+  k.out = pooled, k.B = B, k.HW = HW, k.A = A, k.P = P;
+  k.splits = pool_splits(B, A);
+  k.noise_u = noise_u, k.noise_scale = noise_scale, k.similarity = similarity;
+  k.pose = pose, k.presence = presence, k.feature = feature, k.absence = absence;
+  h.m = m, h.xm = xm;
+  int rc = check(k);
+  if (rc) return rc;
+  if (!scae_capsule_head_conv_supported(HW, A, P, C)) return SCAE_ERR_UNSUPPORTED;
+  if (images < 0 || images > 2) return SCAE_ERR_BAD_ARG;
+  h.G = images ? images : pooled_images(B, k.splits);
+  if (pooled_fwd_lds(h.G, HW, A / k.splits, P, C).total * sizeof(float) > kPooledLdsMax)
+    return SCAE_ERR_UNSUPPORTED;
+  SCAE_REQUIRE(x && w && m && xm && pooled && pose && presence && (feature || P == 8));
+  SCAE_REQUIRE((((size_t)x | (size_t)w) & 15) == 0);
+  return SCAE_OK;
+}
+
+int pooled_bwd_args(PooledArgs &h, const float *x, const float *w, const float *bias, int C,
+                    const float *m, const float *pooled, const float *noise_u,
+                    float noise_scale, int similarity, const float *g_pose,
+                    const float *g_presence, const float *g_feature, const float *g_feature2,
+                    float *gs, float *v, float *dl, float *xdl, float *brow, int B, int HW,
+                    int A, int P) {
+  h = PooledArgs{};
+  PoolArgs &k = h.k;
+  k.cx = x, k.cw = w, k.cb = bias, k.C = C;
+  k.B = B, k.HW = HW, k.A = A, k.P = P;
+  k.splits = pool_splits(B, A);
+  k.noise_u = noise_u, k.noise_scale = noise_scale, k.similarity = similarity;
+  k.pooled = pooled, k.g_pose = g_pose, k.g_presence = g_presence, k.g_feature = g_feature;
+  k.g_feature2 = g_feature2;
+  h.m = const_cast<float *>(m), h.G = 1, h.gs = gs, h.v = v, h.dl = dl, h.xdl = xdl;
+  h.brow = brow;
+  int rc = check(k);
+  if (rc) return rc;
+  if (!scae_capsule_head_conv_supported(HW, A, P, C)) return SCAE_ERR_UNSUPPORTED;
+  if (pooled_bwd_lds(HW, A / k.splits, P, C).total * sizeof(float) > kPooledLdsMax)
+    return SCAE_ERR_UNSUPPORTED;
+  SCAE_REQUIRE(x && w && m && pooled && gs && v && dl && xdl && brow);
+  SCAE_REQUIRE((((size_t)x | (size_t)w) & 15) == 0);
+  return SCAE_OK;
+}
+}
+
+extern "C" int scae_capsule_head_pooled_preferred(int B, int HW, int A, int P, int C) {
+  if (!scae_capsule_head_conv_preferred(B, HW, A, P, C)) return 0;
+  const int Ag = A / pool_splits(B, A);
+  return pooled_fwd_lds(2, HW, Ag, P, C).total * sizeof(float) <= kPooledLdsMax &&
+         pooled_bwd_lds(HW, Ag, P, C).total * sizeof(float) <= kPooledLdsMax &&
+         pooled_grads_lds(HW, A, P) * sizeof(float) <= kPooledLdsMax && P <= NT;
+}
+
+extern "C" int scae_capsule_head_pooled_fwd_f32(
+    const float *x, const float *w, const float *bias, int C, float *m, float *xm,
+    const float *noise_u, float noise_scale, int similarity, float *pooled, float *pose,
+    float *presence, float *feature, float *absence, int B, int HW, int A, int P, int images,
+    void *stream) {
+  PooledArgs h;
+  int rc = pooled_fwd_args(h, x, w, bias, C, m, xm, noise_u, noise_scale, similarity, pooled,
+                           pose, presence, feature, absence, B, HW, A, P, images);
+  if (rc) return rc;
+  const int S = h.k.splits;
+  scae::launch(pooled_fwd_kernel, dim3((B + h.G - 1) / h.G * S), dim3(NT),
+               pooled_fwd_lds(h.G, HW, A / S, P, C).total * sizeof(float), (hipStream_t)stream,
+               h);
+  return scae_launch_status();
+}
+
+extern "C" int scae_capsule_head_pooled_fwd_tc_f32(
+    const float *x, const float *w, const float *bias, int C, float *m, float *xm,
+    const float *noise_u, float noise_scale, int similarity, float *pooled, float *pose,
+    float *presence, float *feature, float *absence, int B, int HW, int A, int P, int images,
+    const float *logits, const float *w1, const float *b1, const float *w2, const float *b2,
+    float *raw, float *templates, float *color, int Ct, int hw, int F, int H1,
+    int template_nonlin, int color_nonlin, void *stream) {
+  PooledArgs h;
+  int rc = pooled_fwd_args(h, x, w, bias, C, m, xm, noise_u, noise_scale, similarity, pooled,
+                           pose, presence, feature, absence, B, HW, A, P, images);
+  if (rc) return rc;
+  SCAE_REQUIRE(feature);
+  scae_tc::TcArgs tk{};
+  tk.logits = logits, tk.feature = feature, tk.w1 = w1, tk.b1 = b1, tk.w2 = w2, tk.b2 = b2;
+  tk.raw = raw, tk.templates = templates, tk.color = color;
+  tk.B = B, tk.M = A, tk.C = Ct, tk.hw = hw, tk.F = F, tk.H1 = H1;
+  tk.tnl = template_nonlin, tk.cnl = color_nonlin;
+  tk.splits = scae_tc::tc_splits(B, A);
+  rc = scae_tc::check(tk);
+  if (rc) return rc;
+  SCAE_REQUIRE(logits && w1 && b1 && w2 && b2 && raw && templates && color);
+  const int S = h.k.splits;
+  if (tk.splits != S || F != P - 8 || S == 1) return SCAE_ERR_UNSUPPORTED;
+  const size_t lp = pooled_fwd_lds(h.G, HW, A / S, P, C).total,
+               lt = scae_tc::lds_floats(A / S, Ct, F, H1, false);
+  scae::launch(pooled_tc_fwd_kernel, dim3((B + h.G - 1) / h.G * S), dim3(NT),
+               (lp > lt ? lp : lt) * sizeof(float), (hipStream_t)stream, h, tk);
+  return scae_launch_status();
+}
+
+extern "C" int scae_capsule_head_pooled_bwd_f32(
+    const float *x, const float *w, const float *bias, int C, const float *m,
+    const float *pooled, const float *noise_u, float noise_scale, int similarity,
+    const float *g_pose, const float *g_presence, const float *g_feature,
+    const float *g_feature2, float *gs, float *v, float *dl, float *xdl, float *brow, int B,
+    int HW, int A, int P, void *stream) {
+  PooledArgs h;
+  int rc = pooled_bwd_args(h, x, w, bias, C, m, pooled, noise_u, noise_scale, similarity,
+                           g_pose, g_presence, g_feature, g_feature2, gs, v, dl, xdl, brow, B,
+                           HW, A, P);
+  if (rc) return rc;
+  scae::launch(pooled_bwd_kernel, dim3(B * h.k.splits), dim3(NT),
+               pooled_bwd_lds(HW, A / h.k.splits, P, C).total * sizeof(float),
+               (hipStream_t)stream, h);
+  return scae_launch_status();
+}
+
+extern "C" int scae_capsule_head_pooled_bwd_tc_f32(
+    const float *x, const float *w, const float *bias, int C, const float *m,
+    const float *pooled, const float *noise_u, float noise_scale, int similarity,
+    const float *g_pose, const float *g_presence, const float *g_feature, float *gs, float *v,
+    float *dl, float *xdl, float *brow, int B, int HW, int A, int P, const float *logits,
+    const float *feature, const float *w1, const float *b1, const float *w2, const float *b2,
+    const float *color, const float *g_templates, const float *g_raw, float *g_logits,
+    float *tc_g_feature, float *partial, int Ct, int hw, int F, int H1, int template_nonlin,
+    int color_nonlin, void *stream) {
+  PooledArgs h;
+  int rc = pooled_bwd_args(h, x, w, bias, C, m, pooled, noise_u, noise_scale, similarity,
+                           g_pose, g_presence, g_feature, tc_g_feature, gs, v, dl, xdl, brow, B,
+                           HW, A, P);
+  if (rc) return rc;
+  scae_tc::TcArgs tk;
+  rc = scae_tc::bwd_args(tk, logits, feature, w1, b1, w2, b2, color, g_templates, g_raw, g_logits,
+                         tc_g_feature, partial, B, A, Ct, hw, F, H1, template_nonlin,
+                         color_nonlin);
+  if (rc) return rc;
+  const int S = h.k.splits;
+  if (tk.splits != S || F != P - 8 || S == 1) return SCAE_ERR_UNSUPPORTED;
+  const size_t lp = pooled_bwd_lds(HW, A / S, P, C).total,
+               lt = scae_tc::lds_floats(A / S, Ct, F, H1, true);
+  const int nA = B * S;
+  scae::launch(pooled_tc_bwd_kernel, dim3(nA + scae_tc::bwd_elementwise_blocks(tk)), dim3(NT),
+               (lp > lt ? lp : lt) * sizeof(float), (hipStream_t)stream, h, tk, nA);
+  return scae_launch_status();
+}
+
+extern "C" int scae_capsule_head_pooled_grads_f32(
+    const float *w, const float *m, const float *xm, const float *gs, const float *v,
+    const float *dl, const float *xdl, const float *brow, const float *gate, float *dx,
+    float *raw, float *part, int B, int HW, int A, int P, int C, int S, void *stream) {
+  if (B <= 0 || HW <= 0 || A <= 0 || P < 2 || S <= 0 || B % S) return SCAE_ERR_BAD_ARG;
+  if (HW > 32 || C < 64 || C % 64 || P > NT) return SCAE_ERR_UNSUPPORTED;
+  const size_t lds = pooled_grads_lds(HW, A, P);
+  if (lds * sizeof(float) > kPooledLdsMax) return SCAE_ERR_UNSUPPORTED;
+  SCAE_REQUIRE(w && m && xm && gs && v && dl && xdl && brow && dx && part);
+  SCAE_REQUIRE((((size_t)w | (size_t)xm | (size_t)xdl | (size_t)v) & 15) == 0);
+  PooledGradArgs k{};
+  k.w = w, k.m = m, k.xm = xm, k.gs = gs, k.v = v, k.dl = dl, k.xdl = xdl, k.brow = brow;
+  k.gate = gate, k.dx = dx, k.raw = raw, k.part = part;
+  k.B = B, k.HW = HW, k.A = A, k.P = P, k.C = C, k.S = S, k.gsz = B / S;
+  const int nch = C / 64;
+  k.nW = S * A * nch;
+  scae::launch(pooled_grads_kernel, dim3(k.nW + B * nch), dim3(NT), lds * sizeof(float),
+               (hipStream_t)stream, k);
+  return scae_launch_status();
+}
diff --git a/torch_scae_amd/ops.py b/torch_scae_amd/ops.py
--- a/torch_scae_amd/ops.py
+++ b/torch_scae_amd/ops.py
@@ -1157,7 +1157,7 @@
 
 
 def _conv1x1_bwd(x, weight, dy, gate=None, outs=None, raw_sum=None,
-                 defer=False):
+                 defer=False, pooled=None):
     B, HW, C = x.shape
     AP = weight.shape[0]
     gsz = max(d for d in range(1, B + 1)
@@ -1165,17 +1165,22 @@
     S, kper, slab = B // gsz, HW * gsz, AP * C + AP
     part = torch.empty(S, slab, device=x.device, dtype=x.dtype)
     dx = torch.empty_like(x)
-    dgrad = _gemm_desc(_p(dy), _p(weight), _p(dx), 1, B * HW, C, AP, True, AP,
-                       0, False, C, 0, C, 0)
-    raw = None
-    if gate is not None:
-        raw = torch.empty_like(x)
-        dgrad.mask, dgrad.ldmask, dgrad.c_nomask = gate.data_ptr(), C, \
-            raw.data_ptr()
-    _gemm_pair(
-        _gemm_desc(_p(dy), _p(x), _p(part), S, AP, C, kper, False, AP,
-                   kper * AP, False, C, kper * C, C, slab,
-                   asum=_off(part, AP * C), asum_b=slab), dgrad, x)
+    raw = torch.empty_like(x) if gate is not None else None
+    if pooled is not None:
+        A, *parts = pooled
+        _lib.call("scae_capsule_head_pooled_grads_f32", _p(weight),
+                  *[_p(t) for t in parts], _p(gate), _p(dx), _p(raw), _p(part),
+                  B, HW, A, AP // A, C, S, _stream(x))
+    else:
+        dgrad = _gemm_desc(_p(dy), _p(weight), _p(dx), 1, B * HW, C, AP, True,
+                           AP, 0, False, C, 0, C, 0)
+        if gate is not None:
+            dgrad.mask, dgrad.ldmask, dgrad.c_nomask = gate.data_ptr(), C, \
+                raw.data_ptr()
+        _gemm_pair(
+            _gemm_desc(_p(dy), _p(x), _p(part), S, AP, C, kper, False, AP,
+                       kper * AP, False, C, kper * C, C, slab,
+                       asum=_off(part, AP * C), asum_b=slab), dgrad, x)
     jobs = [dict(partial=part, shapes=[tuple(weight.shape), (AP,)], outs=outs,
                  defer=defer)]
     if raw_sum is not None:
@@ -1227,7 +1232,14 @@
             _stream(x))
     if _lib.load().scae_capsule_head_conv_preferred(B, HW, n_caps, P, C) and \
             (x.data_ptr() | weight.data_ptr()) % 16 == 0:
-        y = new(B, HW, n_caps * P)
+        if not _bf16() and _lib.load().scae_capsule_head_pooled_preferred(
+                B, HW, n_caps, P, C):
+            m, xm = new(B, n_caps, HW), new(B, n_caps, C)
+            state, form = (m, xm, bias), "scae_capsule_head_pooled_fwd"
+            lead, head = (_p(m), _p(xm)), (*head[:-1], _POOLED_IMAGES, head[-1])
+        else:
+            y = new(B, HW, n_caps * P)
+            state, form, lead = (y,), "scae_capsule_head_conv_fwd", (_p(y),)
         offer = _plan().offers.get("tc_fwd")
         if offer is not None and feature is not None and offer.result is None \
                 and offer.M == n_caps and offer.F == F and offer.ok:
@@ -1235,20 +1247,41 @@
             templates = new(B, n_caps, offer.C, *offer.hw)
             color = new(B, n_caps, offer.C)
             if _lib.try_call(
-                    "scae_capsule_head_conv_fwd_tc_f32", _p(x), _p(weight),
-                    _p(bias), C, _p(y), *head[:-1],
+                    form + "_tc_f32", _p(x), _p(weight),
+                    _p(bias), C, *lead, *head[:-1],
                     *[_p(t) for t in offer.params], _p(raw), _p(templates),
                     _p(color), offer.C, offer.hw[0] * offer.hw[1], F, offer.H1,
                     *offer.codes, head[-1]):
                 offer.result, offer.feature = (raw, templates, color), feature
-                return y, pooled, pose, presence, feature, absence
+                return state, pooled, pose, presence, feature, absence
             offer.ok = False
-        _lib.call("scae_capsule_head_conv_fwd_f32", _p(x), _p(weight),
-                  _p(bias), C, _p(y), *head)
+        _lib.call(form + "_f32", _p(x), _p(weight), _p(bias), C, *lead, *head)
     else:
         y = _conv1x1_fwd(x, weight, bias)
         _lib.call("scae_capsule_head_fwd_f32", _p(y), *head)
-    return y, pooled, pose, presence, feature, absence
+        state = (y,)
+    return state, pooled, pose, presence, feature, absence
+
+
+_POOLED_IMAGES = int(__import__("os").environ.get("SCAE_HEAD_POOLED_IMAGES", "0"))
+
+
+def _capsule_head_bwd_form(x, weight, state, pooled, noise_u, noise_scale,
+                           similarity, A):
+    B, HW, C = x.shape
+    front = (_p(pooled), _p(noise_u), noise_scale, similarity)
+    if len(state) == 1:
+        dy = torch.empty_like(state[0])
+        return "scae_capsule_head_bwd", (_p(state[0]), *front), (_p(dy),), \
+            dy, None
+    m, xm, bias = state
+    P = weight.shape[0] // A
+    new = lambda *shape: torch.empty(*shape, device=x.device, dtype=x.dtype)
+    outs = (new(B, A, P - 1), new(B, A, C), new(B, A, HW), new(B, A, C),
+            new(B, A * P))
+    return "scae_capsule_head_pooled_bwd", \
+        (_p(x), _p(weight), _p(bias), C, _p(m), *front), \
+        tuple(_p(t) for t in outs), None, (A, m, xm, *outs)
 
 
 class _CapsuleHead(torch.autograd.Function):
@@ -1262,12 +1295,12 @@
         P = weight.shape[0] // n_caps
         F = P - 8
         new = lambda *shape: torch.empty(*shape, device=x.device, dtype=x.dtype)
-        y, pooled, pose, presence, feature, absence = _capsule_head_fwd(
+        state, pooled, pose, presence, feature, absence = _capsule_head_fwd(
             x, weight, bias, noise_u, n_caps, noise_scale, similarity)
-        ctx.save_for_backward(x, weight, y, pooled,
+        ctx.save_for_backward(x, weight, pooled, *state,
                               *([noise_u] if noise_u is not None else []))
         ctx.meta = (n_caps, float(noise_scale), int(similarity),
-                    noise_u is not None)
+                    noise_u is not None, len(state))
         ctx.set_materialize_grads(False)
         if feature is None:
             feature = new(B, n_caps, 0)
@@ -1277,16 +1310,18 @@
 
     @_bwd
     def backward(ctx, g_pose, g_presence, g_feature, _g_absence):
-        x, weight, y, pooled = ctx.saved_tensors[:4]
-        A, noise_scale, similarity, has_noise = ctx.meta
-        noise_u = ctx.saved_tensors[4] if has_noise else None
+        x, weight, pooled = ctx.saved_tensors[:3]
+        A, noise_scale, similarity, has_noise, n_state = ctx.meta
+        state = ctx.saved_tensors[3:3 + n_state]
+        noise_u = ctx.saved_tensors[3 + n_state] if has_noise else None
         B, HW, C = x.shape
-        dy = torch.empty_like(y)
-        _lib.call("scae_capsule_head_bwd_f32", _p(y), _p(pooled), _p(noise_u),
-                  noise_scale, similarity, _p(_c(g_pose)), _p(_c(g_presence)),
-                  _p(_c(g_feature)), None, _p(dy), B, HW, A,
+        form, front, outs, dy, parts = _capsule_head_bwd_form(
+            x, weight, state, pooled, noise_u, noise_scale, similarity, A)
+        _lib.call(form + "_f32", *front, _p(_c(g_pose)), _p(_c(g_presence)),
+                  _p(_c(g_feature)), None, *outs, B, HW, A,
                   weight.shape[0] // A, _stream(x))
-        return (*_conv1x1_bwd(x, weight, dy), None, None, None, None)
+        return (*_conv1x1_bwd(x, weight, dy, pooled=parts), None, None, None,
+                None)
 
 
 def capsule_head(x, weight, bias, n_caps, noise_u=None, noise_scale=0.,
@@ -1316,14 +1351,14 @@
         F = P - 8
         noise_u = _c(noise_u)
         new = lambda *shape: torch.empty(*shape, device=x.device, dtype=x.dtype)
-        y, pooled, pose, presence, feature, absence = _capsule_head_fwd(
+        state, pooled, pose, presence, feature, absence = _capsule_head_fwd(
             x, att_w2, att_b.contiguous(), noise_u, n_caps, noise_scale,
             similarity)
-        ctx.save_for_backward(image, *acts, *wds, x, att_w2, y, pooled,
+        ctx.save_for_backward(image, *acts, *wds, x, att_w2, pooled, *state,
                               *([noise_u] if noise_u is not None else []))
         ctx.meta = (tuple(strides), [tuple(w.shape) for w in weights], n_caps,
                     float(noise_scale), int(similarity), noise_u is not None,
-                    tuple(post_bias.shape), tuple(att_w.shape))
+                    tuple(post_bias.shape), tuple(att_w.shape), len(state))
         ctx.slots = [_slot(t, ctx) for t in (post_bias, att_w, att_b, *wb)]
         ctx.refs = [tuple(t.shape) for t in wb]
         ctx.set_materialize_grads(False)
@@ -1341,17 +1376,18 @@
     @_bwd
     def backward(ctx, g_pose, g_presence, g_feature, g_twin, _g_absence):
         (strides, wshapes, A, noise_scale, similarity, has_noise, pb_shape,
-         attw_shape) = ctx.meta
+         attw_shape, n_state) = ctx.meta
         L = len(strides)
         saved = ctx.saved_tensors
         image, acts, wds = saved[0], saved[1:1 + L], saved[1 + L:2 * L]
-        x, att_w2, y, pooled = saved[2 * L:2 * L + 4]
-        noise_u = saved[2 * L + 4] if has_noise else None
+        x, att_w2, pooled = saved[2 * L:2 * L + 3]
+        state = saved[2 * L + 3:2 * L + 3 + n_state]
+        noise_u = saved[2 * L + 3 + n_state] if has_noise else None
         B, HW, C = x.shape
-        dy = torch.empty_like(y)
         P_ = att_w2.shape[0] // A
-        head = (_p(y), _p(pooled), _p(noise_u), noise_scale, similarity,
-                _p(_c(g_pose)), _p(_c(g_presence)))
+        form, front, outs, dy, parts = _capsule_head_bwd_form(
+            x, att_w2, state, pooled, noise_u, noise_scale, similarity, A)
+        head = (*front, _p(_c(g_pose)), _p(_c(g_presence)))
         parked, carried = ctx.plan.take("tc_bwd"), False
         if parked is not None:
             mine = [t for t in (g_twin, g_feature) if t is not None
@@ -1359,17 +1395,17 @@
             rc = _lib.ERR_UNSUPPORTED
             if len(mine) == 1 and parked.bm == (B, A):
                 other = g_feature if mine[0] is g_twin else g_twin
-                rc = _lib.load().scae_capsule_head_bwd_tc_f32(
-                    *head, _p(_c(other)), _p(dy), B, HW, A, P_, *parked.ptrs,
+                rc = getattr(_lib.load(), form + "_tc_f32")(
+                    *head, _p(_c(other)), *outs, B, HW, A, P_, *parked.ptrs,
                     *parked.dims, _stream(x))
             if rc == _lib.ERR_UNSUPPORTED:
                 parked.launch_alone()
             else:
-                _lib.check(rc, "scae_capsule_head_bwd_tc_f32")
+                _lib.check(rc, form + "_tc_f32")
                 carried = True
         if not carried:
-            _lib.call("scae_capsule_head_bwd_f32", *head, _p(_c(g_feature)),
-                      _p(_c(g_twin)), _p(dy), B, HW, A, P_, _stream(x))
+            _lib.call(form + "_f32", *head, _p(_c(g_feature)),
+                      _p(_c(g_twin)), *outs, B, HW, A, P_, _stream(x))
         act = acts[-1]
         g_attw = _grad_out(ctx.slots[1], x, attw_shape)
         g_attb = _grad_out(ctx.slots[2], x, (att_w2.shape[0],))
@@ -1378,7 +1414,8 @@
                                      outs=[g_attw, g_attb],
                                      raw_sum=(pb_shape, g_pb),
                                      defer=all(sl is not None
-                                               for sl in ctx.slots[:3]))
+                                               for sl in ctx.slots[:3]),
+                                     pooled=parts)
         gws, gbs = _conv_stack_bwd(
             image, acts, wds, strides, wshapes, dpre.view(act.shape),
             lambda i: _grad_out(ctx.slots[3 + i], image, ctx.refs[i]),
diff --git a/torch_scae_amd/step_plan.py b/torch_scae_amd/step_plan.py
--- a/torch_scae_amd/step_plan.py
+++ b/torch_scae_amd/step_plan.py
@@ -20,7 +20,8 @@
     ("tc_fwd", Ride(
         "the colour MLP's forward (K10)",
         carriers=("_PartEncoder.forward",), scope="offer",
-        abi="scae_capsule_head_conv_fwd_tc_f32")),
+        abi="scae_capsule_head_conv_fwd_tc_f32 / "
+            "scae_capsule_head_pooled_fwd_tc_f32")),
     ("logprob_fwd", Ride(
         "the reconstruction likelihood's forward (K1)",
         carriers=("_SetEncoder.forward",), scope="offer",
@@ -45,7 +46,8 @@
         "the colour MLP's backward (K10)",
         carriers=("_PartEncoder.backward",),
         readers=("_CapsuleHead.backward",),
-        abi="scae_capsule_head_bwd_tc_f32")),
+        abi="scae_capsule_head_bwd_tc_f32 / "
+            "scae_capsule_head_pooled_bwd_tc_f32")),
     ("reduce", Ride(
         "the output attention's partial-row reduction",
         carriers=("_PartEncoder.backward", "_ConvStack.backward"),
```

New measurement: 253,200. 3.1% lower.
